# Tyler-Sch/pyruhvro

Measured on AMD Instinct MI355X. Metric: Avro records/sec -> Arrow (direct decode, input and output resident in HBM), higher is better.
Workload: dtype u8

## Files before the change

include/ruhvro_hip.h:

```cpp
#ifndef RUHVRO_HIP_H
#define RUHVRO_HIP_H
#include <stddef.h>
#include <stdint.h>
#include "arrow_c_abi.h"

#ifdef __cplusplus
extern "C" {
#endif

#define RH_ABI_VERSION 7

#define RH_OK 0
#define RH_ERR_SCHEMA 1
#define RH_ERR_DECODE 2
#define RH_ERR_RUNTIME 3
#define RH_ERR_ARGUMENT 4

typedef struct rh_schema rh_schema;

rh_schema* rh_schema_compile(const char* json, size_t len, char** err);
void rh_schema_free(rh_schema* s);

rh_schema* rh_schema_project(const rh_schema* s, const char* const* names, uint32_t n_names, char** err);

// ... 10 lines not shown

typedef struct {
  int32_t device;
  int32_t flags;
  void* stream;
  const int32_t* devices;
  uint32_t n_devices;
  uint32_t struct_size;
  uint64_t chunk_rows;
  rh_stats* device_stats;
  const uint64_t* ready;
  uint64_t* gathered;
} rh_opts;

#define RH_KERNEL_AUTO 0
#define RH_KERNEL_GENERIC 1
#define RH_KERNEL_SPECIALIZED 2
#define RH_ASYNC 8
#define RH_TWO_PASS 16
#define RH_SINGLE_PASS 32

struct rh_stats {
  uint64_t records;
  uint64_t input_bytes;
  uint64_t output_bytes;
  uint32_t chunks;
  uint32_t blocks;
  float pack_ms;
  float h2d_ms;
  float size_kernel_ms;
  float scan_kernel_ms;
  float emit_kernel_ms;
  float d2h_ms;
  float total_ms;
  uint32_t specialized;
  uint32_t lds_bytes;
};

int rh_decode(const rh_schema* s, const uint8_t* const* ptrs, const uint64_t* lens,
              uint64_t n, uint64_t num_chunks, const rh_opts* opts,
              struct ArrowArray* out_chunks, uint32_t* out_k, rh_stats* stats, char** err);

int rh_decode_packed(const rh_schema* s, const uint8_t* data, const uint64_t* offsets,
                     uint64_t n, uint64_t num_chunks, const rh_opts* opts,
                     struct ArrowArray* out_chunks, uint32_t* out_k, rh_stats* stats, char** err);

typedef struct rh_device_result rh_device_result;
int rh_decode_device(const rh_schema* s, const void* d_data, const void* d_offsets,
                     uint64_t data_len, uint64_t n, uint64_t num_chunks, const rh_opts* opts,
                     rh_device_result** out, rh_stats* stats, char** err);
int rh_device_result_wait(rh_device_result* r, rh_stats* stats, char** err);
uint32_t rh_device_result_chunks(const rh_device_result* r);
uint64_t rh_device_result_output_bytes(const rh_device_result* r);
int rh_device_result_export(rh_device_result* r, uint32_t chunk, struct ArrowDeviceArray* out);
uint32_t rh_device_result_buffers(rh_device_result* r, uint32_t chunk, uint64_t* ptrs, uint64_t* sizes, uint32_t cap);
int rh_device_result_to_host(rh_device_result* r, struct ArrowArray* out_chunks, char** err);
void rh_device_result_free(rh_device_result* r);

char* rh_schema_kernel_source(const rh_schema* s);
char* rh_schema_kernel_key(const rh_schema* s, int encode);
char* rh_schema_encode_kernel_source(const rh_schema* s);
int rh_schema_prebuild(const rh_schema* s, int* cached, char** err);
int rh_schema_kernels_ready(const rh_schema* s, int encode, long timeout_ms, char** err);

char* rh_schema_lean_kernel_source(const rh_schema* s);
char* rh_schema_lean_kernel_key(const rh_schema* s);
int rh_schema_lean_ready(const rh_schema* s, long timeout_ms, char** err);
int rh_schema_lean_state(const rh_schema* s, int device);
enum {
  RH_LEAN_CALLS = 0,
  RH_LEAN_PROBES = 1,
  RH_LEAN_PROBES_CLEAN = 2,
  RH_LEAN_PROBES_DIRTY = 3,
  RH_LEAN_FALLBACKS = 4,
  RH_LEAN_RERUNS = 5,
  RH_LEAN_NEED_RANGED = 6,
  RH_LEAN_NEED_WIDE_INDEX = 7,
  RH_LEAN_TWO_PASS_REPEATS = 8,
  RH_LEAN_CAPACITY_TAILS = 9,
  RH_LEAN_ASYNC_SETTLED = 10,
  RH_LEAN_COUNT = 11
};
uint32_t rh_lean_counters(uint64_t* out, uint32_t n);

int rh_encode(const rh_schema* s, const struct ArrowArray* batch, const struct ArrowSchema* batch_schema,
              uint64_t num_chunks, const rh_opts* opts, struct ArrowArray* out_chunks, uint32_t* out_k,
              rh_stats* stats, char** err);

typedef struct rh_device_encoded rh_device_encoded;
int rh_encode_device(const rh_schema* s, const struct ArrowArray* batch, const struct ArrowSchema* batch_schema,
                     uint64_t num_chunks, const rh_opts* opts, rh_device_encoded** out, rh_stats* stats, char** err);
uint32_t rh_device_encoded_chunks(const rh_device_encoded* r);
uint64_t rh_device_encoded_output_bytes(const rh_device_encoded* r);
int rh_device_encoded_export(rh_device_encoded* r, uint32_t chunk, struct ArrowDeviceArray* out);
int rh_device_encoded_to_host(rh_device_encoded* r, struct ArrowArray* out_chunks, char** err);
void rh_device_encoded_free(rh_device_encoded* r);

enum {
  RH_CTR_FUSED_CALLS = 0,
  RH_CTR_TWO_SYNC_CALLS = 1,
  RH_CTR_CAPACITY_RETRIES = 2,
  RH_CTR_WIDE_FALLBACKS = 3,
  RH_CTR_OFFSET32_ERRORS = 4,
  RH_CTR_SPLIT_CALLS = 5,
  RH_CTR_SINGLE_PASS_CALLS = 6,
  RH_CTR_SINGLE_PASS_FAILOVERS = 7,
  RH_CTR_BACKGROUND_COMPILES = 8,
  RH_CTR_TILES = 9,
  RH_CTR_CAREFUL_TILES = 10,
  RH_CTR_OVER_WINDOW_TILES = 11,
  RH_CTR_REWALKED_WAVES = 12,
  RH_CTR_SUBTILED_TILES = 13,
  RH_CTR_RANGED_RETRIES = 14,
  RH_CTR_TOLERANT_CALLS = 15,
  RH_CTR_TOLERANT_REPAIRS = 16,
  RH_CTR_COUNT = 17
};
uint32_t rh_engine_counters(uint64_t* out, uint32_t n);

int rh_schema_placeholder(const rh_schema* s, const uint8_t** bytes, uint64_t* len);
typedef struct rh_record_errors rh_record_errors;
uint64_t rh_record_errors_count(const rh_record_errors* e);
int rh_record_errors_get(const rh_record_errors* e, uint64_t i, uint64_t* index, int* code, const char** message);
void rh_record_errors_free(rh_record_errors* e);
int rh_validate(const rh_schema* s, const uint8_t* const* ptrs, const uint64_t* lens, uint64_t n, const rh_opts* opts,
                uint64_t max_errors, rh_record_errors** out, uint64_t* total_bad, char** err);
int rh_validate_packed(const rh_schema* s, const uint8_t* data, const uint64_t* offsets, uint64_t n, const rh_opts* opts,
                       uint64_t max_errors, rh_record_errors** out, uint64_t* total_bad, char** err);
int rh_validate_device(const rh_schema* s, const void* d_data, const void* d_offsets, uint64_t data_len, uint64_t n,
                       const rh_opts* opts, uint64_t max_errors, rh_record_errors** out, uint64_t* total_bad, char** err);
int rh_decode_tolerant(const rh_schema* s, const uint8_t* const* ptrs, const uint64_t* lens, uint64_t n, uint64_t num_chunks,
                       const rh_opts* opts, struct ArrowArray* out_chunks, uint32_t* out_k, rh_stats* stats, char** err,
                       uint64_t max_errors, rh_record_errors** errors);
int rh_decode_packed_tolerant(const rh_schema* s, const uint8_t* data, const uint64_t* offsets, uint64_t n, uint64_t num_chunks,
                              const rh_opts* opts, struct ArrowArray* out_chunks, uint32_t* out_k, rh_stats* stats, char** err,
                              uint64_t max_errors, rh_record_errors** errors);
int rh_decode_device_tolerant(const rh_schema* s, const void* d_data, const void* d_offsets, uint64_t data_len, uint64_t n,
                              uint64_t num_chunks, const rh_opts* opts, rh_device_result** out, rh_stats* stats, char** err,
                              uint64_t max_errors, rh_record_errors** errors);

typedef struct rh_container_info rh_container_info;
int rh_container_scan(const uint8_t* data, uint64_t len, rh_container_info** info, char** err);
const char* rh_container_info_schema(const rh_container_info* i, uint64_t* len);
const char* rh_container_info_codec(const rh_container_info* i);
const uint8_t* rh_container_info_sync(const rh_container_info* i);
uint64_t rh_container_info_blocks(const rh_container_info* i);
uint64_t rh_container_info_records(const rh_container_info* i);
int rh_container_info_table(const rh_container_info* i, const uint64_t** start, const uint64_t** end, const uint64_t** first);
uint32_t rh_container_info_metadata_count(const rh_container_info* i);
int rh_container_info_metadata_get(const rh_container_info* i, uint32_t k, const char** key, const uint8_t** value, uint64_t* value_len);
void rh_container_info_free(rh_container_info* i);
int rh_decode_blocks(const rh_schema* s, const uint8_t* data, uint64_t len, const uint64_t* start, const uint64_t* end,
                     const uint64_t* first, uint64_t nb, uint64_t num_chunks, const rh_opts* opts, struct ArrowArray* out_chunks,
                     uint32_t* out_k, rh_stats* stats, char** err);
int rh_decode_blocks_device(const rh_schema* s, const uint8_t* data, uint64_t len, const uint64_t* start, const uint64_t* end,
                            const uint64_t* first, uint64_t nb, uint64_t num_chunks, const rh_opts* opts, rh_device_result** out,
                            rh_stats* stats, char** err);
float rh_split_last_ms(void);

uint64_t rh_bench_gather(const uint8_t* const* ptrs, const uint64_t* lens, uint64_t n, uint32_t shards,
                         uint32_t threads_per_shard, int pinned, uint32_t reps, double* best_ms);
uint32_t rh_numa_nodes(void);

uint32_t rh_selftest_pool(uint32_t workers, uint32_t phases, uint32_t max_tasks);

void rh_free_string(char* s);
// ... 10 lines not shown
```

pyruhvro_amd/_build.py:

```python
from __future__ import annotations

import os
import subprocess
import sysconfig

HERE = os.path.dirname(os.path.abspath(__file__))
CSRC = os.path.join(HERE, "csrc")
ROOT = os.path.dirname(HERE)
LIB = os.path.join(HERE, "libruhvro_hip.so")
EXT = os.path.join(HERE, "_pyruhvro.so")

LIB_SOURCES = ["kernels.hip", "encode.hip", "validate.hip", "container.hip", "engine_tolerant.cpp", "engine_container.cpp", "container_scan.cpp", "engine.cpp", "engine_pools.cpp", "engine_kernels.cpp", "engine_device_call.cpp", "engine_host.cpp",
               "engine_export.cpp", "engine_encode.cpp", "schema.cpp", "specialize.cpp", "rtc_compile.cpp", "kernel_jobs.cpp"]
HELPER = os.path.join(HERE, "rh_kcompile")
EMBED = ["program.h", "walk.h", "kernel_common.h", "spec_body.h", "encode.h", "encode_walk.h", "encode_spec.h", "walk_drop.h", "spec_flat.h", "walk_resolve.h"]
LIB_DEPS = LIB_SOURCES + EMBED + ["engine_internal.h", "specialize.h", "rtc_compile.h", "kernel_jobs.h", "kcompile_main.cpp", "schema.h", "validate.h", "container.h", "container_scan.h", "json.hpp", "../../include/ruhvro_hip.h", "../../include/arrow_c_abi.h"]


def _stale(target: str, deps) -> bool:
    if not os.path.exists(target):
        return True
    t = os.path.getmtime(target)
    return any(os.path.getmtime(os.path.join(CSRC, d)) > t for d in deps)


def _embed_headers() -> None:
    out = ["// generated by pyruhvro_amd/_build.py from " + ", ".join(EMBED) + " -- do not edit"]
    for h in EMBED:
        text = open(os.path.join(CSRC, h)).read()
        assert ")RHX\"" not in text
        out.append("static const char kHdr_%s[] = R\"RHX(%s)RHX\";" % (h.replace(".", "_"), text))
    path = os.path.join(CSRC, "embedded_headers.inc")
    new = "\n".join(out) + "\n"
    if not os.path.exists(path) or open(path).read() != new:
        open(path, "w").write(new)


def _prune_kernel_cache() -> None:
    d = os.path.join(HERE, "_kcache")
    if os.path.isdir(d):
        for f in os.listdir(d):
            if f.endswith((".hsaco", ".tmp", ".ok", ".lock", ".src", ".err")):
                try:
                    os.remove(os.path.join(d, f))
                except OSError:
                    pass


def _compile_objects(verbose: bool = False):
    from concurrent.futures import ThreadPoolExecutor
    objdir = os.path.join(HERE, "build")
    os.makedirs(objdir, exist_ok=True)
    inc = ["-I", os.path.join(ROOT, "include")]
    clang = "/opt/rocm/lib/llvm/bin/clang++"
    jobs = []
    for src in LIB_SOURCES:
        obj = os.path.join(objdir, os.path.splitext(src)[0] + ".o")
        if src.endswith(".hip") or not os.path.exists(clang):
            cmd = ["hipcc", "--offload-arch=gfx950", "-O3", "-std=c++17", "-fPIC", "-w"] + inc + ["-c", os.path.join(CSRC, src), "-o", obj]
        else:
            cmd = [clang, "-O3", "-std=c++17", "-fPIC", "-w", "-D__HIP_PLATFORM_AMD__", "-I", "/opt/rocm/include"] + inc + \
                  ["-c", os.path.join(CSRC, src), "-o", obj]
        jobs.append((cmd, obj))

    def run(job):
        if verbose:
            print(" ".join(job[0]))
        subprocess.check_call(job[0])
        return job[1]

    with ThreadPoolExecutor(max_workers=min(len(jobs), os.cpu_count() or 2)) as ex:
        return list(ex.map(run, jobs))


def build_lib(force: bool = False, verbose: bool = False) -> str:
    if force or _stale(LIB, LIB_DEPS):
        _embed_headers()
        objs = _compile_objects(verbose)
        cmd = ["hipcc", "--offload-arch=gfx950", "-fPIC", "-shared"] + objs + ["-o", LIB + ".tmp", "-lpthread", "-ldl"]
        if verbose:
            print(" ".join(cmd))
        subprocess.check_call(cmd)
        os.replace(LIB + ".tmp", LIB)
        for o in objs:
            os.remove(o)
        build_helper(verbose)
        _prune_kernel_cache()
    elif not os.path.exists(HELPER):
        build_helper(verbose)
    return LIB


def build_helper(verbose: bool = False) -> str:
    _embed_headers()
    cmd = ["g++", "-O2", "-std=c++17", "-w", os.path.join(CSRC, "kcompile_main.cpp"), os.path.join(CSRC, "rtc_compile.cpp"),
           "-o", HELPER + ".tmp", "-ldl", "-lpthread"]
    if verbose:
        print(" ".join(cmd))
# ... 68 lines not shown
```

pyruhvro_amd/cabi.py:

```python
from __future__ import annotations

import ctypes as C
import os
from collections import namedtuple
from typing import List, Optional

import numpy as np
import pyarrow as pa

_HERE = os.path.dirname(os.path.abspath(__file__))
LIB_PATH = os.environ.get("RUHVRO_HIP_LIB") or os.path.join(_HERE, "libruhvro_hip.so")

RH_OK, RH_ERR_SCHEMA, RH_ERR_DECODE, RH_ERR_RUNTIME, RH_ERR_ARGUMENT = range(5)


class RhStats(C.Structure):
    _fields_ = [("records", C.c_uint64), ("input_bytes", C.c_uint64), ("output_bytes", C.c_uint64),
                ("chunks", C.c_uint32), ("blocks", C.c_uint32), ("pack_ms", C.c_float), ("h2d_ms", C.c_float),
                ("size_kernel_ms", C.c_float), ("scan_kernel_ms", C.c_float), ("emit_kernel_ms", C.c_float),
                ("d2h_ms", C.c_float), ("total_ms", C.c_float), ("specialized", C.c_uint32), ("lds_bytes", C.c_uint32)]

    def as_dict(self):
        return {n: getattr(self, n) for n, _ in self._fields_}

# ... 239 lines not shown
KERNEL_AUTO, KERNEL_GENERIC, KERNEL_SPECIALIZED = 0, 1, 2
RH_TWO_PASS = 16
RH_SINGLE_PASS = 32
RH_ASYNC = 8


def kernel_source(schema_json: str, columns=None, reader_schema=None) -> str:
    L = lib()
    p = L.rh_schema_kernel_source(Schema.get(schema_json, columns, reader_schema).handle)
    if not p:
        raise RuntimeError("rh_schema_kernel_source failed")
    try:
        return C.string_at(p).decode()
    finally:
        L.rh_free_string(p)


def kernel_key(schema_json: str, encode: bool = False, columns=None, reader_schema=None) -> str:
    L = lib()
    p = L.rh_schema_kernel_key(Schema.get(schema_json, columns, reader_schema).handle, 1 if encode else 0)
    if not p:
        raise RuntimeError("rh_schema_kernel_key failed")
    try:
        return C.string_at(p).decode()
    finally:
        L.rh_free_string(p)


LEAN_COUNTERS = ("lean_calls", "probes", "probes_clean", "probes_dirty", "fallbacks", "reruns", "need_ranged", "need_wide_index",
                 "two_pass_repeats", "capacity_tails", "async_settled")
LEAN_NONE, LEAN_UNDECIDED, LEAN_LEAN, LEAN_WIDE = -1, 0, 1, 2


def _lean_sym(name: str, restype, argtypes):
    f = getattr(lib(), name, None)
    if f is not None:
        f.restype, f.argtypes = restype, argtypes
    return f


def _lean_string(name: str, schema_json: str, columns=None, reader_schema=None):
    f = _lean_sym(name, C.c_void_p, [C.c_void_p])
    p = f(Schema.get(schema_json, columns, reader_schema).handle) if f else None
    if not p:
        return None
    try:
        return C.string_at(p).decode()
    finally:
        lib().rh_free_string(p)


def lean_kernel_source(schema_json: str, columns=None, reader_schema=None):
    return _lean_string("rh_schema_lean_kernel_source", schema_json, columns, reader_schema)


def lean_kernel_key(schema_json: str, columns=None, reader_schema=None):
    return _lean_string("rh_schema_lean_kernel_key", schema_json, columns, reader_schema)


def lean_state(schema_json: str, device: int = 0, columns=None, reader_schema=None) -> int:
    f = _lean_sym("rh_schema_lean_state", C.c_int, [C.c_void_p, C.c_int])
    return int(f(Schema.get(schema_json, columns, reader_schema).handle, device)) if f else LEAN_NONE


def lean_ready(schema_json: str, timeout_ms: int = 0) -> bool:
    f = _lean_sym("rh_schema_lean_ready", C.c_int, [C.c_void_p, C.c_long, C.POINTER(C.c_char_p)])
    if f is None:
        return False
    err = C.c_char_p()
    rc = f(Schema.get(schema_json).handle, int(timeout_ms), C.byref(err))
    if rc == -1:
        _raise(RH_ERR_RUNTIME, err)
    return rc == 1


def lean_counters() -> dict:
    f = _lean_sym("rh_lean_counters", C.c_uint32, [C.POINTER(C.c_uint64), C.c_uint32])
    buf = (C.c_uint64 * len(LEAN_COUNTERS))()
    if f is not None:
        assert f(buf, len(LEAN_COUNTERS)) == len(LEAN_COUNTERS)
    return {name: int(buf[i]) for i, name in enumerate(LEAN_COUNTERS)}


def encode_kernel_source(schema_json: str) -> str:
    L = lib()
    p = L.rh_schema_encode_kernel_source(Schema.get(schema_json).handle)
    if not p:
        raise RuntimeError("rh_schema_encode_kernel_source failed")
    try:
        return C.string_at(p).decode()
    finally:
        L.rh_free_string(p)


def prebuild(schema_json: str, columns=None, reader_schema=None) -> bool:
    L = lib()
    cached = C.c_int()
    err = C.c_char_p()
    rc = L.rh_schema_prebuild(Schema.get(schema_json, columns, reader_schema).handle, C.byref(cached), C.byref(err))
    if rc != RH_OK:
        _raise(rc, err)
    return bool(cached.value)


def kernels_ready(schema_json: str, encode: bool = False, timeout_ms: int = 0, columns=None, reader_schema=None) -> bool:
    err = C.c_char_p()
    rc = lib().rh_schema_kernels_ready(Schema.get(schema_json, columns, reader_schema).handle, 1 if encode else 0, int(timeout_ms), C.byref(err))
    if rc < 0:
        _raise(RH_ERR_RUNTIME, err)
    return rc == 1


def shard_chunks(n: int, num_chunks: int, n_shards: int, shard: int):
    c0, c1, r0, r1 = C.c_uint32(), C.c_uint32(), C.c_uint64(), C.c_uint64()
    lib().rh_shard_chunks(n, num_chunks, n_shards, shard, C.byref(c0), C.byref(c1), C.byref(r0), C.byref(r1))
    return c0.value, c1.value, r0.value, r1.value


def decode_packed(data: np.ndarray, offsets: np.ndarray, schema_json: str, num_chunks: int,
                  device: int = -1, want_stats: bool = False, kernel: int = KERNEL_AUTO, devices=None, *, columns=None, reader_schema=None):
    L = lib()
    s = Schema.get(schema_json, columns, reader_schema)
    data = np.ascontiguousarray(data, dtype=np.uint8)
    offsets = np.ascontiguousarray(offsets, dtype=np.uint64)
    n = len(offsets) - 1
    k = L.rh_clamp_chunks(n, num_chunks)
    arr = (ArrowArray * k)()
    out_k = C.c_uint32()
    st = RhStats()
    err = C.c_char_p()
    opts, keep = make_opts(device, kernel, None, devices)
    rc = L.rh_decode_packed(s.handle, data.ctypes.data, offsets.ctypes.data, n, num_chunks, C.byref(opts), arr,
                            C.byref(out_k), C.byref(st), C.byref(err))
    if rc != RH_OK:
        _raise(rc, err)
    out = _import_chunks(arr, out_k.value, s.arrow_schema)
    if not want_stats:
        return out
    d = st.as_dict()
    if devices:
        d["device_stats"] = [x.as_dict() for x in keep["device_stats"]]
    return out, d


def decode_slices(ptrs: np.ndarray, lens: np.ndarray, schema_json: str, num_chunks: int,
                  device: int = -1, want_stats: bool = False, kernel: int = KERNEL_AUTO, devices=None, *, columns=None, reader_schema=None):
    L = lib()
    s = Schema.get(schema_json, columns, reader_schema)
    ptrs = np.ascontiguousarray(ptrs, dtype=np.uint64)
    lens = np.ascontiguousarray(lens, dtype=np.uint64)
    n = len(ptrs)
    k = L.rh_clamp_chunks(n, num_chunks)
    arr = (ArrowArray * k)()
    out_k = C.c_uint32()
    st = RhStats()
    err = C.c_char_p()
    opts, keep = make_opts(device, kernel, None, devices)
    rc = L.rh_decode(s.handle, ptrs.ctypes.data, lens.ctypes.data, n, num_chunks, C.byref(opts), arr,
                     C.byref(out_k), C.byref(st), C.byref(err))
    if rc != RH_OK:
        _raise(rc, err)
    out = _import_chunks(arr, out_k.value, s.arrow_schema)
    return (out, st.as_dict()) if want_stats else out


RecordError = namedtuple("RecordError", ["index", "message"])
# ... 391 lines not shown
```

pyruhvro_amd/csrc/engine.cpp:

```cpp
#include "engine_internal.h"

#include <sched.h>

using namespace rhe;

bool stats_line_on() {
  static const bool on = [] { const char* e = std::getenv("RUHVRO_HIP_STATS"); return e && *e && *e != '0'; }();
  return on;
}
void stats_json(std::string& o, const rh_stats& st) {
  char buf[512];
  std::snprintf(buf, sizeof buf,
                "{\"records\": %llu, \"input_bytes\": %llu, \"output_bytes\": %llu, \"chunks\": %u, \"blocks\": %u, \"pack_ms\": %.4f, "
                "\"h2d_ms\": %.4f, \"size_kernel_ms\": %.4f, \"scan_kernel_ms\": %.4f, \"emit_kernel_ms\": %.4f, \"d2h_ms\": %.4f, "
                "\"total_ms\": %.4f, \"specialized\": %u, \"lds_bytes\": %u}",
                (unsigned long long)st.records, (unsigned long long)st.input_bytes, (unsigned long long)st.output_bytes, st.chunks,
                st.blocks, st.pack_ms, st.h2d_ms, st.size_kernel_ms, st.scan_kernel_ms, st.emit_kernel_ms, st.d2h_ms, st.total_ms,
                st.specialized, st.lds_bytes);
  o += buf;
}
void stats_line(const char* entry, int rc, const rh_stats& st, const rh_opts* opts, const rh_stats* shards) {
  std::string o = "{\"ruhvro_hip\": \"";
  o += entry;
  o += "\", \"rc\": " + std::to_string(rc) + ", \"stats\": ";
// ... 198 lines not shown
  return RH_OK;
}

int rh_decode_device(const rh_schema* s, const void* d_data, const void* d_offsets, uint64_t data_len, uint64_t n,
                     uint64_t num_chunks, const rh_opts* opts, rh_device_result** out, rh_stats* stats, char** err) {
  if (!s || !out) return RH_ERR_ARGUMENT;
  return guarded(err, [&] {
    require_device();
    Timer t;
    rh_opts pub;
    if (opts) { pub = *opts; pub.flags &= kPublicFlags; }
    *out = decode_device_impl(const_cast<rh_schema*>(s), (const uint8_t*)d_data, (const uint64_t*)d_offsets, data_len,
                              n, num_chunks, opts ? &pub : nullptr, stats);
    if (stats) stats->total_ms = t.ms();
    return RH_OK;
  });
}

char* rh_schema_kernel_source(const rh_schema* s) {
  if (!s) return nullptr;
  try {
    return dup_msg(rh::generate_kernel_source(*s->cs));
  } catch (...) {
    return nullptr;
  }
}

char* rh_schema_kernel_key(const rh_schema* s, int encode) {
  if (!s) return nullptr;
  try {
    if (encode && (!s->cs->encode_unsupported.empty() || s->cs->projected)) return nullptr;
    const std::string src = encode ? rh::generate_encode_source(*s->cs) : rh::generate_kernel_source(*s->cs);
    return dup_msg(rh::kernel_cache_key(src, encode != 0));
  } catch (...) {
    return nullptr;
  }
}

char* rh_schema_lean_kernel_source(const rh_schema* s) {
  if (!s) return nullptr;
  try {
    const std::string src = rh::generate_lean_source(*s->cs);
    return src.empty() ? nullptr : dup_msg(src);
  } catch (...) {
    return nullptr;
  }
}

char* rh_schema_lean_kernel_key(const rh_schema* s) {
  if (!s) return nullptr;
  try {
    const std::string src = rh::generate_lean_source(*s->cs);
    return src.empty() ? nullptr : dup_msg(rh::kernel_cache_key(src, false));
  } catch (...) {
    return nullptr;
  }
}

int rh_schema_lean_ready(const rh_schema* s, long timeout_ms, char** err) {
  if (!s) return -1;
  try {
    if (!rh::schema_has_lean(*s->cs)) return -2;
    rh::KernelImage im[rh::KP_COUNT];
    rh::kernel_images(s->images, *s->cs, rh::kLeanParts, rh::CP_CACHED_ONLY, im);
    std::string why;
    const int rc = rh::kernel_images_wait(s->images, rh::kLeanParts, timeout_ms, &why);
    if (rc < 0 && err) *err = dup_msg(why);
    return rc;
  } catch (const std::exception& e) {
    if (err) *err = dup_msg(e.what());
    return -1;
  }
}

int rh_schema_lean_state(const rh_schema* cs_, int device) {
  rh_schema* s = const_cast<rh_schema*>(cs_);
  if (!s) return -1;
  if (!rh::schema_has_lean(*s->cs)) return -1;
  std::lock_guard<std::mutex> g(s->mu);
  auto it = s->spec.find(device);
  return (it == s->spec.end() || !it->second) ? 0 : it->second->lean_state;
}

char* rh_schema_encode_kernel_source(const rh_schema* s) {
  if (!s || !s->cs->encode_unsupported.empty() || s->cs->projected) return nullptr;
  try {
    return dup_msg(rh::generate_encode_source(*s->cs));
  } catch (...) {
    return nullptr;
  }
}

int rh_schema_prebuild(const rh_schema* s, int* cached, char** err) {
  if (!s) return RH_ERR_ARGUMENT;
  return guarded(err, [&] {
    const bool fused = env_long("RUHVRO_HIP_PREBUILD_FUSED", 1, 0, 1) != 0;
    const bool ranged = env_long("RUHVRO_HIP_PREBUILD_RANGED", 1, 0, 1) != 0;
    const bool lean = env_long("RUHVRO_HIP_PREBUILD_LEAN", 0, 0, 1) != 0;
    const unsigned parts = (rh::kDecodeParts & ~(fused ? 0u : (1u << rh::KP_FUSED)) & ~(ranged ? 0u : ((1u << rh::KP_SIZE_R) | (1u << rh::KP_EMIT_R)))) |
                           ((s->cs->encode_unsupported.empty() && !s->cs->wide && !s->cs->projected) ? rh::kEncodeParts : 0u) |
                           (lean ? rh::kLeanParts : 0u);
    rh::KernelImage im[rh::KP_COUNT];
    const unsigned started = rh::kernel_images(s->images, *s->cs, parts, rh::CP_BLOCKING, im);
    for (int p = 0; p < rh::KP_COUNT; p++) {
      if (!(parts & (1u << p)) || im[p].state == rh::IMG_NONE) continue;
      if (im[p].state != rh::IMG_READY) throw std::runtime_error(std::string(rh::kernel_part_entry(p)) + ": " + (im[p].why.empty() ? "kernel image missing" : im[p].why));
    }
    if (cached) *cached = started == 0 ? 1 : 0;
    return RH_OK;
  });
}

int rh_schema_kernels_ready(const rh_schema* s, int encode, long timeout_ms, char** err) {
  if (!s) return -1;
  try {
    if (encode && s->cs->projected) {
      if (err) *err = dup_msg(s->cs->resolved ? "a resolved schema is decode only" : "a projected schema is decode only");
      return -1;
    }
    const unsigned parts = encode ? rh::kEncodeParts : ((1u << rh::KP_SIZE) | (1u << rh::KP_EMIT));
    rh::KernelImage im[rh::KP_COUNT];
    rh::kernel_images(s->images, *s->cs, parts, rh::CP_CACHED_ONLY, im);
    std::string why;
    const int rc = rh::kernel_images_wait(s->images, parts, timeout_ms, &why);
    if (rc < 0 && err) *err = dup_msg(why);
    return rc;
  } catch (const std::exception& e) {
    if (err) *err = dup_msg(e.what());
    return -1;
  }
}

uint32_t rh_device_result_chunks(const rh_device_result* r) { return r ? r->k : 0; }

uint64_t rh_device_result_output_bytes(const rh_device_result* r) {
  if (!r) return 0;
  try {
    settle(const_cast<rh_device_result*>(r));
    if (!r->parts.empty()) {
      uint64_t sum = 0;
      for (auto& p : r->parts) { p->tables(); sum += p->output_bytes; }
      return sum;
    }
    const_cast<rh_device_result*>(r)->tables();
  } catch (...) {
    return 0;
  }
  return r->output_bytes;
}

int rh_device_result_wait(rh_device_result* r, rh_stats* stats, char** err) {
  if (!r) return RH_ERR_ARGUMENT;
  return guarded(err, [&] {
    settle(r);
    if (stats && r->has_stats) *stats = r->st;
    return RH_OK;
  });
}

int rh_device_result_export(rh_device_result* r, uint32_t chunk, struct ArrowDeviceArray* out) {
  if (!r || !out || chunk >= r->k) return RH_ERR_ARGUMENT;
  std::memset(out, 0, sizeof *out);
  try {
    settle(r);
    rh_device_result* owner = r;
    for (size_t g = 0; g < r->parts.size(); g++)
      if (chunk >= r->part_chunk0[g] && chunk < r->part_chunk0[g] + r->parts[g]->k) { owner = r->parts[g].get(); chunk -= r->part_chunk0[g]; break; }
    owner->tables();
    export_chunk(*owner, chunk, owner->arena.ptr(), nullptr, &out->array);
  } catch (const DecodeError&) {
    return RH_ERR_DECODE;
  } catch (...) {
    return RH_ERR_RUNTIME;
  }
  out->device_id = r->device;
  out->device_type = ARROW_DEVICE_ROCM;
  out->sync_event = nullptr;
  return RH_OK;
}

uint32_t rh_device_result_buffers(rh_device_result* r, uint32_t chunk, uint64_t* ptrs, uint64_t* sizes, uint32_t cap) {
  if (!r || chunk >= r->k) return 0;
  try {
    settle(r);
// ... 51 lines not shown
```

pyruhvro_amd/csrc/engine_device_call.cpp:

```cpp
#include "engine_internal.h"

using namespace rhe;

struct rh_decode_call {
  rh_schema* s;
  const CompiledSchema& cs;
  const uint8_t* d_data;
  const uint64_t* d_offsets;
  uint64_t data_len, n, num_chunks;
  rh_opts opts;
  bool want_stats;
  rh_stats st;
  rh_device_result& r;
  HostProf hp;
  int device = 0;
  hipStream_t stream = nullptr;
  ChunkGeo geo_v;
  const ChunkGeo* geo = nullptr;
  uint32_t k = 1;
  int K = 0, nnodes = 0, nbuf = 0;
  const DeviceProgram* dp = nullptr;
  const SpecKernel* sk = nullptr;
  hipFunction_t size_r = nullptr, emit_r = nullptr;
  hipFunction_t size_f = nullptr, emit_f = nullptr;
  hipFunction_t lean_size = nullptr, lean_emit = nullptr;
  bool lean = false;
  bool probing = false;
  uint32_t probe_token = 0;
  Lease probe_ws, probe_host;
  std::unique_ptr<CtrlLease> probe_ctrl;
  uint64_t narrow_rows = 0, tile = 0, bpc64 = 0, payload = 0;
  uint32_t nblocks = 0;
  uint64_t o_null = 0, o_tot = 48, ctrl_bytes = 0;
  uint32_t null_slots = rh::kNullSlots;
  Lease ws, hctrl, dtab, prof_buf;
  std::unique_ptr<CtrlLease> ctrl;
  rh::KParams P;
  uint32_t lds_bytes = 0, emit_lds = 0;
  bool profile = false;
  Events ev;
  std::vector<uint64_t> totals;
  uint64_t n_entries = 0, tab_bytes = 0;
  uint64_t* d_sizes = nullptr;
  uint64_t exact = 0;
  bool child_bitmaps = false, fused = false, timed_size = false;
  bool range_of_host_call = false;
  bool single = false;
  std::vector<uint64_t> caps;
  uint64_t arena_cap = 0, o_tick = 0;
  Lease lookback, hcaps;
  double basis = 0;
  bool settled = false;
  bool async = false;
  DoneEvent done;
  hipEvent_t start_after = nullptr, sized = nullptr;
  bool published = false;
  uint32_t token = 0;
  uint64_t o_flag_h = 0;

  rh_decode_call(rh_schema* s_, const uint8_t* data, const uint64_t* offs, uint64_t dl, uint64_t n_, uint64_t nc, const rh_opts* o,
               bool stats, const ChunkGeo* g, rh_device_result& res)
      : s(s_), cs(*s_->cs), d_data(data), d_offsets(offs), data_len(dl), n(n_), num_chunks(nc), opts(o ? *o : default_opts()),
        want_stats(stats), r(res) {
    std::memset(&st, 0, sizeof st);
    if (g) { geo_v = *g; geo = &geo_v; range_of_host_call = true; }
    opts.devices = nullptr; opts.n_devices = 0; opts.device_stats = nullptr; opts.ready = nullptr; opts.gathered = nullptr;
  }

  Lease arena_lease(uint64_t bytes) {
    r.arena_host = false;
    if ((opts.flags & RH_INTERNAL_HOST_ARENA) && !child_bitmaps && env_long("RUHVRO_HIP_HOST_ARENA", 1, 0, 1) != 0) {
      Block b = pin_pool().try_get(bytes, device);
      if (b.p) {
        r.arena_host = true;
        return Lease(pin_pool(), b);
      }
      pin_pool().prefetch(bytes + bytes / 16, device, pinned_budget_left());
    }
    return Lease(dev_pool(), bytes, device);
  }

  void check_bad(const uint8_t* h) {
    unsigned long long fb = *(const unsigned long long*)h;
    if (!fb) return;
    const uint64_t rec = ~fb;
    uint64_t c = r.sz ? std::min<uint64_t>(rec / r.sz, k - 1) : 0;
    uint64_t b = c * bpc64 + (rec - c * r.sz) / tile;
    rh::ErrInfo ei;
    HIPCHK(hipMemcpy(&ei, P.errinfo + b, sizeof ei, hipMemcpyDeviceToHost));
    throw RecordDecodeError(format_error(ei));
  }

  void learn_unsized_tiles() {
    if (timed_size || single || n == 0) return;
    const uint32_t* stw = (const uint32_t*)(hctrl.ptr() + 32);
    count(RH_CTR_OVER_WINDOW_TILES, stw[1]); count(RH_CTR_SUBTILED_TILES, stw[3]);
    if (stw[1]) s->ranged_calls.store(kRangedKeep, std::memory_order_relaxed);
    else { uint32_t v = s->ranged_calls.load(std::memory_order_relaxed); if (v) s->ranged_calls.compare_exchange_weak(v, v - 1, std::memory_order_relaxed); }
  }

  void layout_host() {
    r.data_bytes = totals;
    for (auto t : totals)
      if (t > 0x7FFFFFFFull) {
        count(RH_CTR_OFFSET32_ERRORS);
        throw DecodeError("offset overflow: a chunk's column exceeds the 2^31-1 limit of 32-bit Arrow offsets");
      }
    if (sk)
      for (int d = 1; d < cs.ndom; d++)
        for (uint32_t c = 0; c < k; c++)
          if (totals[(size_t)(d - 1) * k + c] >= narrow_rows) {
            if (lean) lean_count(LC_NEED_WIDE_INDEX);
            throw NeedWideIndex();
          }
    r.fill_tables();
    exact = r.output_bytes;
  }

  void launch_tail(bool offsets_done) {
    if (nbuf > 0 && (child_bitmaps || !offsets_done) &&
        rh_launch_init(P.bufptr, d_sizes, dp->desc, (uint32_t)nbuf, k, P.first_bad, stream)) throw HipError("k_init launch failed");
    if (n > 0) {
      emit_lds = lds_bytes;
      if (sk ? launch_module(emit_f, P, nblocks, (uint32_t)tile, emit_lds, stream, ev.at(3), P.ranged ? nullptr : ev.at(4))
             : (cs.projected ? rh_launch_emit_drop : rh_launch_emit)(&P, emit_lds, stream, ev.at(3), ev.at(4)))
        throw HipError("k_emit launch failed");
      if (P.ranged && launch_module(emit_r, P, nblocks + (P.worklist ? rh::kBigFront : 0u), (uint32_t)tile, emit_lds, stream, nullptr, ev.at(4))) throw HipError("k_emit (ranged) launch failed");
    } else {
      ev.rec(3, stream);
      ev.rec(4, stream);
// ... 52 lines not shown
    const uint64_t rows_lastp = kp == k ? r.rows_last : r.sz;
    const uint32_t tiles_last = (uint32_t)std::min<uint64_t>(per, (rows_lastp + tile - 1) / tile);
    if (per == 0 || tiles_last == 0) return;
    const uint32_t pn = (kp - 1) * per + tiles_last;
    {
      std::lock_guard<std::mutex> g(s->mu);
      SpecKernel& sl = sel();
      if (sl.lean_state == SpecKernel::LS_LEAN || sl.lean_probing) return;
      if (sl.lean_state == SpecKernel::LS_WIDE && sl.lean_wait > 0) { sl.lean_wait--; return; }
      sl.lean_probing = true;
    }
    probing = true;
    const uint64_t q_bsum = align_up(sizeof(rh::ErrInfo) * (uint64_t)pn, kAlign);
    const uint64_t q_flag = align_up(q_bsum + 4ull * std::max(K, 1) * pn, kAlign);
    const uint64_t q_lcnt = align_up(q_flag + 4ull * pn, kAlign);
    const uint64_t q_end = align_up(q_lcnt + 4ull * (uint64_t)((cs.KL + 1) / 2) * pn * tile, kAlign) + kAlign;
    probe_ws = Lease(dev_pool(), q_end, device);
    probe_host = Lease(pin_pool(), 256, device);
    probe_ctrl.reset(new CtrlLease(ctrl_bytes, device, stream));
    void* hdev = nullptr;
    if (hipHostGetDevicePointer(&hdev, probe_host.ptr(), 0) != hipSuccess || !hdev) {
      (void)hipGetLastError();
      probe_abandon();
      return;
    }
    rh::KParams Q = P;
    Q.k = kp; Q.rows_last = rows_lastp; Q.bpc = per; Q.nblocks = pn;
    Q.ranged = 0; Q.worklist = nullptr; Q.bigmark = nullptr; Q.all_careful = 0; Q.lookback = nullptr; Q.caps = nullptr;
    Q.first_bad = (unsigned long long*)probe_ctrl->ptr();
    Q.nullcount = (uint32_t*)(probe_ctrl->ptr() + o_null);
    Q.totals = (uint64_t*)(probe_ctrl->ptr() + o_tot);
    Q.tickets = (uint32_t*)(probe_ctrl->ptr() + o_tick);
    Q.errinfo = (rh::ErrInfo*)probe_ws.ptr();
    Q.blocksum = (uint32_t*)(probe_ws.ptr() + q_bsum);
    Q.blockbase = Q.blocksum;
    Q.tileflag = (uint32_t*)(probe_ws.ptr() + q_flag);
    Q.lanecnt = (uint32_t*)(probe_ws.ptr() + q_lcnt);
    Q.lanecnt32 = nullptr;
    static std::atomic<uint32_t> next_token{0x20000001u};
    probe_token = next_token.fetch_add(1);
    if (probe_token == 0) probe_token = next_token.fetch_add(1);
    *(volatile uint32_t*)(probe_host.ptr() + 48) = 0;
    if (launch_module(lean_size, Q, pn, (uint32_t)tile, lds_bytes, stream) ||
        rh_launch_tile_stats(probe_ctrl->ptr(), Q.tileflag, pn, stream) ||
        rh_launch_publish(probe_ctrl->ptr(), hdev, 12, 0, 12, probe_token, null_slots, stream))
      throw HipError("lean probe launch failed");
  }

  void probe_abandon() noexcept {
    if (!probing) return;
    probing = false;
    std::lock_guard<std::mutex> g(s->mu);
    sel().lean_probing = false;
  }

  void probe_settle() {
    if (!probing) return;
    volatile uint32_t* flag = (volatile uint32_t*)(probe_host.ptr() + 48);
    bool got = true;
    for (uint32_t spins = 0; __atomic_load_n(flag, __ATOMIC_ACQUIRE) != probe_token;) {
      if ((++spins & 0xFFFFu) == 0) {
        const hipError_t q = hipStreamQuery(stream);
        if (q == hipErrorNotReady) continue;
        got = __atomic_load_n(flag, __ATOMIC_ACQUIRE) == probe_token;
        break;
      }
    }
    const uint32_t* h = (const uint32_t*)probe_host.ptr();
    const bool clean = got && h[0] == 0 && h[1] == 0 && h[2] == 0 && h[8] == 0 && h[9] == 0 && h[10] == 0;
    lean_count(LC_PROBES);
    lean_count(clean ? LC_PROBES_CLEAN : LC_PROBES_DIRTY);
    {
      std::lock_guard<std::mutex> g(s->mu);
      SpecKernel& sl = sel();
      sl.lean_probing = false;
      if (clean) sl.lean_state = SpecKernel::LS_LEAN;
      else { sl.lean_state = SpecKernel::LS_WIDE; sl.lean_wait = 64; }
    }
    probing = false;
    if (got) { probe_ws.release(); probe_host.release(); probe_ctrl.reset(); }
  }

  void lean_learn(bool dirty) {
    if (!lean) return;
    std::lock_guard<std::mutex> g(s->mu);
    SpecKernel& sl = sel();
    if (dirty) {
      if (sl.lean_state != SpecKernel::LS_WIDE) {
        sl.lean_backoff = std::min<uint32_t>(1024, std::max<uint32_t>(8, sl.lean_backoff * 2));
        sl.lean_wait = sl.lean_backoff;
        sl.lean_state = SpecKernel::LS_WIDE;
        lean_count(LC_FALLBACKS);
      }
    } else if (sl.lean_state == SpecKernel::LS_LEAN) {
      sl.lean_backoff = 0;
    }
  }

  bool try_single(bool two_sync, long ratio_hook) {
    const bool on = (opts.flags & RH_SINGLE_PASS) != 0 || env_long("RUHVRO_HIP_SINGLE_PASS", kSinglePassDefault, 0, 1) != 0;
    if (!on || range_of_host_call || (opts.flags & (RH_INTERNAL_TWO_PASS | RH_TWO_PASS)) || !sk || K <= 0 || K > 64 || n == 0 || two_sync ||
        ratio_hook >= 0)
      return false;
    if (n_entries > (1u << 16)) return false;
    if (8ull * K * k > 4ull * K * nblocks) return false;
    hipFunction_t fused_fn = sk->fused_fn.load(std::memory_order_acquire);
    if (!fused_fn) {
      if (sk->fused_dead) return false;
      fused_fn = spec_kernel(s, device, compile_policy(opts.flags & 3, n), false, true).fused_fn.load(std::memory_order_acquire);
      if (!fused_fn) return false;
    }
    std::vector<double> per_row;
    {
      std::lock_guard<std::mutex> g(s->mu);
      if ((int)s->per_row.size() != K) return false;
      if (s->single_cooldown > 0) { s->single_cooldown--; return false; }
      per_row = s->per_row;
    }
    const double slack = (double)env_long("RUHVRO_HIP_SINGLE_SLACK_PERMILLE", 1040, 1, 4000) / 1000.0;
    caps.assign((size_t)K * k, 0);
    for (int kk = 0; kk < K; kk++)
      for (uint32_t c = 0; c < k; c++) {
        const uint64_t rows_c = c == k - 1 ? r.rows_last : r.sz;
        uint64_t cap = (uint64_t)(per_row[(size_t)kk] * (double)rows_c * slack) + (slack >= 1.0 ? 4096 : 0);
        uint64_t lim = 0x7FFFFFFFull;
        if (kk < cs.ndom - 1) lim = std::min<uint64_t>(lim, narrow_rows - 1);
        caps[(size_t)kk * k + c] = std::min(cap, lim);
      }
    {
      uint64_t off = 0;
      for (uint32_t c = 0; c < k; c++)
        for (int b = 0; b < nbuf; b++) {
          const rh::BufDesc& d = cs.bufs[b];
          const uint64_t rows0 = c == k - 1 ? r.rows_last : r.sz;
          const uint64_t rows = d.dom == 0 ? rows0 : caps[(size_t)(d.dom - 1) * k + c];
          off += rh::buf_slot_bytes(rh::buf_bytes(d.kind, rows, d.kind == rh::BK_DATA ? caps[(size_t)d.counter * k + c] : 0, nullptr, (uint32_t)d.counter));
        }
      arena_cap = std::max<uint64_t>(off, kAlign);
    }
    count(RH_CTR_SINGLE_PASS_CALLS);
    count(RH_CTR_FUSED_CALLS);
    single = true; fused = true;
    r.arena = Lease(dev_pool(), arena_cap, device);
    lookback = Lease(dev_pool(), std::max<uint64_t>(8ull * K * nblocks, kAlign), device);
    HIPCHK(hipMemsetAsync(lookback.ptr(), 0, 8ull * K * nblocks, stream));
    hcaps = Lease(pin_pool(), 8ull * K * k, device);
    std::memcpy(hcaps.ptr(), caps.data(), 8ull * K * k);
    uint64_t* d_caps = (uint64_t*)P.blocksum;
    HIPCHK(hipMemcpyAsync(d_caps, hcaps.ptr(), 8ull * K * k, hipMemcpyHostToDevice, stream));
    P.lookback = (unsigned long long*)lookback.ptr();
    P.caps = d_caps;
    rh::LParams LP;
    std::memset(&LP, 0, sizeof LP);
    LP.totals = d_caps; LP.desc = dp->desc; LP.sz = r.sz; LP.rows_last = r.rows_last; LP.n = n; LP.k = k;
    LP.nbuf = nbuf; LP.K = K; LP.ndom = cs.ndom; LP.arena = r.arena.ptr(); LP.capacity = r.arena.b.size;
    LP.bufptr = (void**)dtab.ptr(); LP.bufsize = d_sizes; LP.ctrl = P.first_bad; LP.narrow = 0;
    LP.narrow_rows = narrow_rows;
    if (rh_launch_layout(&LP, stream)) throw HipError("k_layout launch failed");
    if (nbuf > 0 && child_bitmaps && rh_launch_init(P.bufptr, d_sizes, dp->desc, (uint32_t)nbuf, k, P.first_bad, stream))
      throw HipError("k_init launch failed");
    const uint64_t tiles_max = std::max<uint64_t>((r.sz + tile - 1) / tile, (r.rows_last + tile - 1) / tile);
    emit_lds = lds_bytes;
    if (launch_module(fused_fn, P, (uint32_t)(tiles_max * k), (uint32_t)tile, emit_lds, stream, ev.at(3), ev.at(4)))
      throw HipError("k_fused launch failed");
    basis = (double)payload + 64.0 * (double)n;
    void* hdev = nullptr;
    if (hipHostGetDevicePointer(&hdev, hctrl.ptr(), 0) == hipSuccess && hdev) {
      static std::atomic<uint32_t> next_token{0x40000001u};
      token = next_token.fetch_add(1);
      if (token == 0) token = next_token.fetch_add(1);
      o_flag_h = align_up(o_null + 4ull * nnodes * k, 8);
      *(volatile uint32_t*)(hctrl.ptr() + o_flag_h) = 0;
      if (rh_launch_publish(ctrl->ptr(), hdev, (uint32_t)(o_null / 4), (uint32_t)(nnodes * (int)k), (uint32_t)(o_flag_h / 4), token, null_slots, stream))
        throw HipError("k_publish launch failed");
      ctrl->b.clean = true;
      published = true;
    } else {
      (void)hipGetLastError();
      HIPCHK(hipMemcpyAsync(hctrl.ptr(), ctrl->ptr(), ctrl_bytes, hipMemcpyDeviceToHost, stream));
      if (async) done.record(device, stream);
    }
    return true;
  }

  void enqueue() {
    Range rk("ruhvro_hip:decode_device (k_size, k_scan, k_layout, k_init, k_emit)");
    if (opts.device >= 0) { HIPCHK(hipSetDevice(opts.device)); device = opts.device; }
    else HIPCHK(hipGetDevice(&device));
    stream = (hipStream_t)opts.stream;
    if ((uintptr_t)d_data & 15) throw std::invalid_argument("device payload pointer must be 16-byte aligned");

    {
      static std::mutex lds_mu;
      static std::vector<int> lds_done;
      std::lock_guard<std::mutex> g(lds_mu);
      if (std::find(lds_done.begin(), lds_done.end(), device) == lds_done.end()) {
        if (rh_set_max_lds(160 * 1024) != 0) throw HipError("cannot raise the dynamic LDS limit of the decode kernels");
        lds_done.push_back(device);
      }
    }

    r.cs = &cs;
    r.device = device;
    r.n = n;
    if (!geo && opts.chunk_rows) {
      if (num_chunks < 1 || num_chunks > 0xFFFFFFFFull || (num_chunks - 1) > n / opts.chunk_rows ||
          (n > 0 && n == (num_chunks - 1) * opts.chunk_rows && num_chunks > 1))
        throw std::invalid_argument("chunk_rows: the n records do not make num_chunks chunks of chunk_rows rows (the last one takes the rest)");
      geo_v.k = (uint32_t)num_chunks;
      geo_v.sz = opts.chunk_rows;
      geo_v.rows_last = n - (num_chunks - 1) * opts.chunk_rows;
      geo_v.payload_bytes = data_len;
      geo = &geo_v;
    }
    k = geo ? geo->k : rh_clamp_chunks(n, num_chunks);
    r.k = k;
    r.sz = geo ? geo->sz : n / k;
    r.rows_last = geo ? geo->rows_last : n - (uint64_t)(k - 1) * r.sz;
    K = cs.K; nnodes = (int)cs.nodes.size(); nbuf = (int)cs.bufs.size();
    dp = &device_program(s, device);

    const int mode = opts.flags & 3;
// ... 152 lines not shown
      const uint64_t capacity = align_up((uint64_t)(ratio * basis * 1.125) + n_entries * kAlign + (1u << 20), kAlign);
      r.arena = arena_lease(capacity);
      rh::LParams LP;
      std::memset(&LP, 0, sizeof LP);
      LP.totals = P.totals; LP.desc = dp->desc; LP.sz = r.sz; LP.rows_last = r.rows_last; LP.n = n; LP.k = k;
      LP.nbuf = nbuf; LP.K = K; LP.ndom = cs.ndom; LP.arena = r.arena.ptr(); LP.capacity = r.arena.b.size;
      LP.bufptr = (void**)dtab.ptr(); LP.bufsize = d_sizes; LP.ctrl = P.first_bad; LP.narrow = sk ? 1u : 0u;
      LP.narrow_rows = narrow_rows;
      if (timed_size && K == 0 && rh_launch_tile_stats(ctrl->ptr(), P.tileflag, nblocks, stream)) throw HipError("k_tile_stats launch failed");
      if ((timed_size && K > 0) ? rh_launch_scan_layout(&P, &LP, stream, ev.at(5), ev.at(2)) : rh_launch_layout(&LP, stream))
        throw HipError("k_scan / k_layout launch failed");
      launch_tail(true);
      hp.mark("layout+emit_launch");
      void* hdev = nullptr;
      static const bool no_publish = env_long("RUHVRO_HIP_NO_PUBLISH", 0, 0, 1) != 0;
      if (!no_publish && hipHostGetDevicePointer(&hdev, hctrl.ptr(), 0) == hipSuccess && hdev) {
        static std::atomic<uint32_t> next_token{1};
        token = next_token.fetch_add(1);
        if (token == 0) token = next_token.fetch_add(1);
        o_flag_h = align_up(o_null + 4ull * nnodes * k, 8);
        *(volatile uint32_t*)(hctrl.ptr() + o_flag_h) = 0;
        if (rh_launch_publish(ctrl->ptr(), hdev, (uint32_t)(o_null / 4), (uint32_t)(nnodes * (int)k), (uint32_t)(o_flag_h / 4), token, null_slots, stream))
          throw HipError("k_publish launch failed");
        ctrl->b.clean = true;
        published = true;
      } else {
        (void)hipGetLastError();
        HIPCHK(hipMemcpyAsync(hctrl.ptr(), ctrl->ptr(), ctrl_bytes, hipMemcpyDeviceToHost, stream));
        if (async) done.record(device, stream);
      }
      hp.mark("d2h_enqueue");
    }
    launch_probe();
  }

  void finish() {
    if (settled) return;
    settled = true;
    HIPCHK(hipSetDevice(device));
    if (fused) {
      if (published) {
        volatile uint32_t* flag = (volatile uint32_t*)(hctrl.ptr() + o_flag_h);
        for (uint32_t spins = 0; __atomic_load_n(flag, __ATOMIC_ACQUIRE) != token;) {
          if ((++spins & 0xFFFFu) == 0) {
            const hipError_t q = hipStreamQuery(stream);
            if (q == hipSuccess) {
              if (__atomic_load_n(flag, __ATOMIC_ACQUIRE) != token) throw HipError("rh_k_publish finished without publishing its token");
              break;
            }
            if (q != hipErrorNotReady) throw HipError(std::string("stream failed while waiting for a decode call: ") + hipGetErrorString(q));
          }
#if defined(__x86_64__)
          __builtin_ia32_pause();
#endif
        }
      } else if (done.e) {
        done.wait();
      } else {
        HIPCHK(hipStreamSynchronize(stream));
      }
      hp.mark("sync");
      probe_settle();
      const uint32_t lflag = *(const uint32_t*)(hctrl.ptr() + 8);
      if (lflag & rh::LF_NEED_RANGED) {
        ctrl->b.clean = published;
        s->ranged_calls.store(kRangedKeep, std::memory_order_relaxed);
        r.arena.release();
        if (lean) { lean_count(LC_NEED_RANGED); lean_learn(true); }
        throw NeedRanged();
      }
      check_bad(hctrl.ptr());
      if (lean && !single) { const uint32_t* stw = (const uint32_t*)(hctrl.ptr() + 32); lean_learn(stw[0] != 0 || stw[2] != 0); }
      if (published && timed_size && !single) {
        const uint32_t* stw = (const uint32_t*)(hctrl.ptr() + 32);
        count(RH_CTR_TILES, nblocks);
        count(RH_CTR_CAREFUL_TILES, stw[0]); count(RH_CTR_OVER_WINDOW_TILES, stw[1]);
        count(RH_CTR_REWALKED_WAVES, stw[2]); count(RH_CTR_SUBTILED_TILES, stw[3]);
        if (stw[1]) s->ranged_calls.store(kRangedKeep, std::memory_order_relaxed);
        else { uint32_t v = s->ranged_calls.load(std::memory_order_relaxed); if (v) s->ranged_calls.compare_exchange_weak(v, v - 1, std::memory_order_relaxed); }
      }
      if (K > 0) std::memcpy(totals.data(), hctrl.ptr() + o_tot, 8ull * K * k);
      if (single) {
        ctrl->b.clean = published;
        if (lflag) {
          if ((lflag & rh::LF_CAPACITY) && env_long("RUHVRO_HIP_SINGLE_SLACK_PERMILLE", 1040, 1, 4000) >= 1000) {
            std::lock_guard<std::mutex> g(s->mu);
            s->single_backoff = std::min<uint32_t>(1024, std::max<uint32_t>(8, s->single_backoff * 2));
            s->single_cooldown = s->single_backoff;
          }
          count(RH_CTR_SINGLE_PASS_FAILOVERS);
          r.arena.release();
          throw NeedTwoPass();
        }
        r.data_bytes = totals;
        r.layout_bytes = caps;
        r.arena_bytes = arena_cap;
        { std::lock_guard<std::mutex> g(s->mu); s->single_backoff = 0; }
      } else if (lflag & rh::LF_CAPACITY) {
        count(RH_CTR_CAPACITY_RETRIES);
        if (lean) lean_count(LC_CAPACITY_TAILS);
        r.arena.release();
        exact_tail();
      } else if (lflag || want_stats) {
        layout_host();
        if (lflag) throw HipError("internal error: layout kernel and host disagree");
        if (r.arena_bytes != std::max<uint64_t>(*(const uint64_t*)(hctrl.ptr() + 16), kAlign)) throw HipError("internal error: device and host arena layouts differ");
      } else {
        r.data_bytes = totals;
        r.arena_bytes = std::max<uint64_t>(*(const uint64_t*)(hctrl.ptr() + 16), kAlign);
      }
    } else {
      count(RH_CTR_TWO_SYNC_CALLS);
      if (timed_size) {
        HIPCHK(hipMemcpyAsync(hctrl.ptr(), ctrl->ptr(), ctrl_bytes, hipMemcpyDeviceToHost, stream));
        HIPCHK(hipStreamSynchronize(stream));
        probe_settle();
        if (*(const uint32_t*)(hctrl.ptr() + 8) & rh::LF_NEED_RANGED) {
          ctrl->b.clean = false;
          s->ranged_calls.store(kRangedKeep, std::memory_order_relaxed);
          throw NeedRanged();
        }
        check_bad(hctrl.ptr());
        std::memcpy(totals.data(), hctrl.ptr() + o_tot, 8ull * K * k);
      }
      exact_tail();
    }
    learn_unsized_tiles();
    if (n > 0 && basis > 0 && !single) {
      const double slots = (double)n_entries * (double)kAlign;
      s->arena_ratio.store(std::max(0.0, (double)r.arena_bytes - slots) / basis + 1e-9);
    }
    if (n > 0 && K > 0 && (int)totals.size() == K * (int)k) {
      std::vector<double> pr((size_t)K, 0.0);
      for (int kk = 0; kk < K; kk++)
        for (uint32_t c = 0; c < k; c++) {
          const uint64_t rows_c = c == k - 1 ? r.rows_last : r.sz;
          if (rows_c) pr[(size_t)kk] = std::max(pr[(size_t)kk], (double)totals[(size_t)kk * k + c] / (double)rows_c);
        }
      std::lock_guard<std::mutex> g(s->mu);
      s->per_row = std::move(pr);
    }
    r.nullcount.assign((size_t)nnodes * k, 0);
    if (published) {
      std::memcpy(r.nullcount.data(), hctrl.ptr() + o_null, 4ull * nnodes * k);
    } else {
      const uint32_t* slots = (const uint32_t*)(hctrl.ptr() + o_null);
      for (size_t e = 0; e < (size_t)nnodes * k; e++) {
        uint32_t sum = 0;
        for (uint32_t sl = 0; sl < null_slots; sl++) sum += slots[e * null_slots + sl];
        r.nullcount[e] = sum;
      }
    }
    hp.mark("host_layout");

    if (profile && sk) {
      unsigned long long hr[64 * 32], h[32] = {0};
      HIPCHK(hipMemcpy(hr, prof_buf.ptr(), sizeof hr, hipMemcpyDeviceToHost));
      for (int r0 = 0; r0 < 64; r0++)
        for (int i = 0; i < 32; i++) h[i] += hr[r0 * 32 + i];
      const double waves = (double)nblocks * 4;
      static const char* names2[] = {"offsets", "stage+barrier", "lane_init", "walk1", "scan", "barrier", "layout", "walk2",
                                     "errors+barrier", "flush"};
      static const char* names1[] = {"ticket+zero+barrier", "offsets+stage+barrier", "size_walk", "wave_scan", "barrier", "lookback(wave0)",
                                     "barrier", "prefix", "emit_walk", "errors+flush"};
      const char* const* names = single ? names1 : names2;
      std::fprintf(stderr, "[ruhvro_hip profile] %s cycles/wave:", single ? "single-pass" : "emit");
// ... 288 lines not shown
```

pyruhvro_amd/csrc/engine_internal.h:

```cpp
#pragma once
#include <hip/hip_runtime_api.h>
#include <dlfcn.h>
#include <pthread.h>

extern "C" hipError_t hipExtModuleLaunchKernel(hipFunction_t f, uint32_t globalWorkSizeX, uint32_t globalWorkSizeY,
                                               uint32_t globalWorkSizeZ, uint32_t localWorkSizeX, uint32_t localWorkSizeY,
                                               uint32_t localWorkSizeZ, size_t sharedMemBytes, hipStream_t hStream,
                                               void** kernelParams, void** extra, hipEvent_t startEvent,
                                               hipEvent_t stopEvent, uint32_t flags);

#include <algorithm>
#include <atomic>
#include <chrono>
#include <cstdio>
#include <cstdlib>
#include <cstring>
#include <functional>
#include <map>
#include <condition_variable>
#include <mutex>
#include <string>
#include <thread>
#include <vector>

// ... 192 lines not shown
  uint64_t cached_ = 0;
};

Pool& dev_pool();
Pool& pin_pool();

struct Lease {
  Pool* pool = nullptr;
  Block b;
  Lease() = default;
  Lease(Pool& p, uint64_t size, int device) : pool(&p), b(p.get(size, device)) {}
  Lease(Pool& p, Block taken) : pool(&p), b(taken) {}
  Lease(const Lease&) = delete;
  Lease& operator=(const Lease&) = delete;
  Lease(Lease&& o) noexcept : pool(o.pool), b(o.b) { o.pool = nullptr; o.b = Block(); }
  Lease& operator=(Lease&& o) noexcept {
    if (this != &o) { release(); pool = o.pool; b = o.b; o.pool = nullptr; o.b = Block(); }
    return *this;
  }
  ~Lease() { release(); }
  void release() { if (pool && b.p) pool->put(b); pool = nullptr; b = Block(); }
  uint8_t* ptr() const { return (uint8_t*)b.p; }
};

class CtrlPool {
 public:
  struct Blk { void* p = nullptr; uint64_t size = 0; int device = 0; hipStream_t stream = nullptr; bool clean = false; };
  Blk get(uint64_t size, int device, hipStream_t stream) {
    size = align_up(std::max<uint64_t>(size, 1), 4096);
    {
      std::lock_guard<std::mutex> g(mu_);
      for (size_t i = 0; i < free_.size(); i++)
        if (free_[i].device == device && free_[i].stream == stream && free_[i].size == size) {
          Blk b = free_[i];
          free_.erase(free_.begin() + (long)i);
          return b;
        }
    }
    Blk b;
    b.size = size; b.device = device; b.stream = stream;
    hipError_t e = hipMalloc(&b.p, size);
    if (e != hipSuccess) throw HipError(std::string("HIP allocation of a control block failed: ") + hipGetErrorString(e));
    e = hipMemsetAsync(b.p, 0, size, stream);
    if (e != hipSuccess) { (void)hipFree(b.p); throw HipError(std::string("hipMemsetAsync failed: ") + hipGetErrorString(e)); }
    return b;
  }
  void put(Blk b) {
    if (!b.p) return;
    if (!b.clean && hipMemsetAsync(b.p, 0, b.size, b.stream) != hipSuccess) { (void)hipFree(b.p); return; }
    b.clean = false;
    Blk drop;
    {
      std::lock_guard<std::mutex> g(mu_);
      free_.push_back(b);
      if (free_.size() > 64) { drop = free_.front(); free_.erase(free_.begin()); }
    }
    if (drop.p) (void)hipFree(drop.p);
  }

 private:
  std::mutex mu_;
  std::vector<Blk> free_;
};
CtrlPool& ctrl_pool();

struct CtrlLease {
  CtrlPool::Blk b;
  CtrlLease(uint64_t size, int device, hipStream_t stream) : b(ctrl_pool().get(size, device, stream)) {}
  CtrlLease(const CtrlLease&) = delete;
  CtrlLease& operator=(const CtrlLease&) = delete;
  ~CtrlLease() { ctrl_pool().put(b); }
  uint8_t* ptr() const { return (uint8_t*)b.p; }
};

struct DeviceProgram {
  rh::Op* prog = nullptr;
  uint32_t* sym_off = nullptr;
  uint8_t* sym_data = nullptr;
  rh::BufDesc* desc = nullptr;
  int32_t* cnt_databuf = nullptr;
};

struct SpecKernel {
  hipModule_t mod[7] = {nullptr, nullptr, nullptr, nullptr, nullptr, nullptr, nullptr};
  hipFunction_t size_fn = nullptr, emit_fn = nullptr;
  std::atomic<hipFunction_t> size_r_fn{nullptr}, emit_r_fn{nullptr};
  std::atomic<bool> ranged_dead{false};
  std::atomic<hipFunction_t> size_l_fn{nullptr}, emit_l_fn{nullptr};
  std::atomic<bool> lean_dead{false};
  enum : int { LS_UNDECIDED = 0, LS_LEAN = 1, LS_WIDE = 2 };
  int lean_state = LS_UNDECIDED;
  uint32_t lean_wait = 0;
  uint32_t lean_backoff = 0;
  bool lean_probing = false;
  std::atomic<hipFunction_t> fused_fn{nullptr};
  std::atomic<bool> fused_dead{false};
  std::atomic<bool> ok{false};
  std::atomic<bool> dead{false};
  std::string why;
};

}

struct rh_schema {
  std::unique_ptr<rh::CompiledSchema> cs;
  std::mutex mu;
  std::map<int, rhe::DeviceProgram> dev;
  std::map<int, std::unique_ptr<rhe::SpecKernel>> spec;
  std::map<int, std::unique_ptr<rhe::SpecKernel>> espec;
  std::shared_ptr<rh::KernelImages> images = rh::new_kernel_images();
  std::atomic<double> arena_ratio{0.0};
  std::vector<double> per_row;
  std::atomic<uint32_t> ranged_calls{0};
  std::vector<uint8_t> placeholder;
  bool placeholder_done = false;
  rh_schema* plain_parent = nullptr;
  uint32_t single_cooldown = 0, single_backoff = 0;
};

namespace rhe {

const DeviceProgram& device_program(rh_schema* s, int device);
uint64_t spec_min_records();
const SpecKernel& spec_kernel(rh_schema* s, int device, rh::CompilePolicy policy, bool encode = false, bool want_fused = false, bool want_ranged = false,
                              bool want_lean = false);
enum LeanCounter { LC_LEAN_CALLS = 0, LC_PROBES, LC_PROBES_CLEAN, LC_PROBES_DIRTY, LC_FALLBACKS, LC_RERUNS, LC_NEED_RANGED, LC_NEED_WIDE_INDEX,
                   LC_TWO_PASS_REPEATS, LC_CAPACITY_TAILS, LC_ASYNC_SETTLED, LC_COUNT };
extern std::atomic<uint64_t> g_lean_counters[LC_COUNT];
inline void lean_count(int which, uint64_t by = 1) { g_lean_counters[which].fetch_add(by, std::memory_order_relaxed); }
rh::CompilePolicy compile_policy(int mode, uint64_t n);
int launch_module(hipFunction_t f, const rh::KParams& P, uint32_t grid, uint32_t block, uint32_t lds, hipStream_t stream,
                  hipEvent_t start = nullptr, hipEvent_t stop = nullptr);
std::string format_error(const rh::ErrInfo& e);

struct Roctx {
  int (*push)(const char*) = nullptr;
  int (*pop)() = nullptr;
  Roctx() {
    const char* e = std::getenv("RUHVRO_HIP_ROCTX");
    const bool want = e && *e && *e != '0';
    for (const char* name : {"librocprofiler-sdk-roctx.so.1", "libroctx64.so.4", "librocprofiler-sdk-roctx.so", "libroctx64.so"}) {
      void* h = dlopen(name, RTLD_LAZY | RTLD_NOLOAD);
      if (!h && want) h = dlopen(name, RTLD_LAZY);
      if (!h) continue;
      push = (int (*)(const char*))dlsym(h, "roctxRangePushA");
      pop = (int (*)())dlsym(h, "roctxRangePop");
      if (push && pop) return;
      push = nullptr; pop = nullptr;
    }
  }
  static const Roctx& get() { static const Roctx r; return r; }
};
struct Range {
  bool on;
  explicit Range(const char* name) : on(Roctx::get().push != nullptr) { if (on) Roctx::get().push(name); }
  ~Range() { if (on) Roctx::get().pop(); }
  Range(const Range&) = delete;
  Range& operator=(const Range&) = delete;
};

struct HostProf {
  bool on;
  std::chrono::steady_clock::time_point t0;
  std::string line;
  HostProf() {
    static const bool e = [] { const char* v = std::getenv("RUHVRO_HIP_HOSTPROF"); return v && *v && *v != '0'; }();
    on = e;
    if (on) t0 = std::chrono::steady_clock::now();
  }
  void mark(const char* what) {
    if (!on) return;
    const auto t = std::chrono::steady_clock::now();
    char buf[64];
    std::snprintf(buf, sizeof buf, " %s=%.1f", what, std::chrono::duration<double, std::micro>(t - t0).count());
    line += buf;
    t0 = t;
  }
  ~HostProf() { if (on) std::fprintf(stderr, "[ruhvro_hip hostprof us]%s\n", line.c_str()); }
};

struct Timeline {
  static bool on() {
    static const bool e = [] { const char* v = std::getenv("RUHVRO_HIP_TIMELINE"); return v && *v && *v != '0'; }();
    return e;
  }
  static std::chrono::steady_clock::time_point& t0() {
    static std::chrono::steady_clock::time_point t = std::chrono::steady_clock::now();
    return t;
  }
  static void start() { if (on()) t0() = std::chrono::steady_clock::now(); }
  static void mark(uint32_t shard, const char* what) {
    if (!on()) return;
    std::fprintf(stderr, "[ruhvro_hip timeline] %8.3f ms  shard %u  %s\n",
                 std::chrono::duration<double, std::milli>(std::chrono::steady_clock::now() - t0()).count(), shard, what);
  }
};

inline rh_opts default_opts() {
  rh_opts o;
  std::memset(&o, 0, sizeof o);
  o.device = -1;
  return o;
}

struct Timer {
  std::chrono::steady_clock::time_point t0 = std::chrono::steady_clock::now();
  float ms() const { return std::chrono::duration<float, std::milli>(std::chrono::steady_clock::now() - t0).count(); }
};
// ... 2 lines not shown

struct rh_decode_call;
struct rh_device_result {
  const rh::CompiledSchema* cs = nullptr;
  int device = 0;
  uint64_t n = 0, sz = 0, rows_last = 0;
  uint32_t k = 1;
  rhe::Lease arena;
  bool arena_host = false;
  uint64_t arena_bytes = 0;
  std::vector<uint64_t> buf_off;
  std::vector<uint64_t> buf_size;
  std::vector<uint64_t> dom_rows;
  std::vector<uint64_t> data_bytes;
  std::vector<uint64_t> layout_bytes;
  std::vector<uint32_t> nullcount;
  uint64_t output_bytes = 0;
  std::mutex tables_mu;
  bool tables_done = false;
  std::unique_ptr<rh_decode_call> pending;
  std::exception_ptr fail;
  rh_stats st;
  bool has_stats = false;
  std::vector<std::unique_ptr<rh_device_result>> parts;
  std::vector<uint32_t> part_chunk0;
  rhe::Lease patched_data, patched_offsets;
  rhe::Lease container_data, container_offsets;
  std::vector<hipEvent_t> join_events;

  rh_device_result();
  ~rh_device_result();
  uint64_t rows(int dom, uint32_t c) const { return dom_rows[(size_t)dom * k + c]; }
  void fill_tables();
  void tables() { std::lock_guard<std::mutex> g(tables_mu); if (!tables_done) fill_tables(); }
};

struct rh_device_encoded {
  int device = 0;
  uint64_t n = 0, sz = 0, rows_last = 0;
  uint32_t k = 1;
  rhe::Lease out;
  uint64_t out_bytes = 0;
  std::vector<uint64_t> ooff;
  std::vector<uint64_t> data_bytes;
  uint64_t exact = 0;
  uint64_t rows(uint32_t c) const { return n == 0 ? 0 : (c == k - 1 ? rows_last : sz); }
};

namespace rhe {

struct Slab {
  std::atomic<int> refs{0};
  void* base = nullptr;
  Block pinned;
  void free_mem() {
    if (pinned.p) {
      pinned_result_bytes().fetch_sub(pinned.size);
      pin_pool().put(pinned);
    } else {
      std::free(base);
    }
    pinned = Block();
    base = nullptr;
  }
  static std::atomic<uint64_t>& pinned_result_bytes() {
    static std::atomic<uint64_t> v{0};
    return v;
  }
};

inline uint64_t pinned_budget_left() {
  static const uint64_t bound = (uint64_t)env_long_early("RUHVRO_HIP_PINNED_RESULT_MB", 4096, 0, 1 << 20) << 20;
  const uint64_t used = Slab::pinned_result_bytes().load();
  return used >= bound ? 0 : bound - used;
}

void export_chunk(const rh_device_result& r, uint32_t c, const uint8_t* base, Slab* slab, ArrowArray* out);
void export_field(const rh::ArrowField& f, ArrowSchema* out);
Slab* slab_from_device(const uint8_t* dptr, uint64_t bytes, int device, hipStream_t stream = nullptr);
int to_host_impl(rh_device_result* r, ArrowArray* out_chunks, hipStream_t stream = nullptr);
void settle(rh_device_result* r);

constexpr long kSinglePassDefault = 0;
constexpr int kPublicFlags = 3 | RH_ASYNC | RH_TWO_PASS | RH_SINGLE_PASS;
constexpr int RH_INTERNAL_HOST_ARENA = 0x200;
constexpr int RH_INTERNAL_TWO_PASS = 0x100;
constexpr long kInternalStreamsDefault = 1;
constexpr long kSplitMinDefault = 1000000;

inline long env_long(const char* name, long dflt, long lo, long hi) {
  const char* e = std::getenv(name);
  if (!e || !*e) return dflt;
  char* end = nullptr;
  const long v = std::strtol(e, &end, 10);
  return (end && *end == 0 && v >= lo && v <= hi) ? v : dflt;
}

struct Events {
  hipEvent_t e[6] = {nullptr, nullptr, nullptr, nullptr, nullptr, nullptr};
  bool on = false;
  int device = 0;
  static std::mutex& mu() { static std::mutex m; return m; }
  static std::map<int, std::vector<hipEvent_t>>& idle() { static auto* v = new std::map<int, std::vector<hipEvent_t>>(); return *v; }
  void init() {
    HIPCHK(hipGetDevice(&device));
    {
      std::lock_guard<std::mutex> g(mu());
      auto& v = idle()[device];
      for (auto& x : e)
        if (!v.empty()) { x = v.back(); v.pop_back(); }
    }
    for (auto& x : e)
      if (!x) HIPCHK(hipEventCreate(&x));
    on = true;
  }
  ~Events() {
    if (!on) return;
    std::lock_guard<std::mutex> g(mu());
    auto& v = idle()[device];
    for (auto& x : e) {
      if (!x) continue;
      if (v.size() < 64) v.push_back(x);
      else (void)hipEventDestroy(x);
    }
  }
  void rec(int i, hipStream_t s) { if (on) HIPCHK(hipEventRecord(e[i], s)); }
  hipEvent_t at(int i) const { return on ? e[i] : nullptr; }
  float ms(int a, int b) {
    float t = 0;
    if (on && hipEventElapsedTime(&t, e[a], e[b]) != hipSuccess) { t = 0; (void)hipGetLastError(); }
    return t;
  }
};

struct DoneEvent {
  hipEvent_t e = nullptr;
  int device = 0;
  static std::mutex& mu() { static std::mutex m; return m; }
  static std::map<int, std::vector<hipEvent_t>>& idle() { static auto* v = new std::map<int, std::vector<hipEvent_t>>(); return *v; }
  void record(int dev, hipStream_t s) {
    device = dev;
    {
      std::lock_guard<std::mutex> g(mu());
      auto& v = idle()[device];
      if (!v.empty()) { e = v.back(); v.pop_back(); }
    }
    if (!e) HIPCHK(hipEventCreateWithFlags(&e, hipEventDisableTiming));
    HIPCHK(hipEventRecord(e, s));
  }
  void wait() { if (e) HIPCHK(hipEventSynchronize(e)); }
  ~DoneEvent() {
    if (!e) return;
    std::lock_guard<std::mutex> g(mu());
    auto& v = idle()[device];
    if (v.size() < 64) v.push_back(e);
    else (void)hipEventDestroy(e);
  }
};

struct ChunkGeo {
  uint64_t sz, rows_last;
  uint32_t k;
  uint64_t payload_bytes;
};

rh_device_result* decode_device_impl1(rh_schema* s, const uint8_t* d_data, const uint64_t* d_offsets, uint64_t data_len,
// ... 49 lines not shown
```

pyruhvro_amd/csrc/engine_kernels.cpp:

```cpp
#include "engine_internal.h"

namespace rhe {

const DeviceProgram& device_program(rh_schema* s, int device) {
  std::lock_guard<std::mutex> g(s->mu);
  auto it = s->dev.find(device);
  if (it != s->dev.end()) return it->second;
  const CompiledSchema& cs = *s->cs;
  DeviceProgram d;
  const size_t pb = cs.prog.size() * sizeof(rh::Op), so = cs.sym_off.size() * 4, sd = cs.sym_data.size(),
               bd = std::max<size_t>(cs.bufs.size(), 1) * sizeof(rh::BufDesc);
  HIPCHK(hipMalloc((void**)&d.prog, pb));
  HIPCHK(hipMalloc((void**)&d.sym_off, so));
  HIPCHK(hipMalloc((void**)&d.sym_data, sd));
  HIPCHK(hipMalloc((void**)&d.desc, bd));
  HIPCHK(hipMemcpy(d.prog, cs.prog.data(), pb, hipMemcpyHostToDevice));
  HIPCHK(hipMemcpy(d.sym_off, cs.sym_off.data(), so, hipMemcpyHostToDevice));
  HIPCHK(hipMemcpy(d.sym_data, cs.sym_data.data(), sd, hipMemcpyHostToDevice));
  if (!cs.bufs.empty()) HIPCHK(hipMemcpy(d.desc, cs.bufs.data(), cs.bufs.size() * sizeof(rh::BufDesc), hipMemcpyHostToDevice));
  std::vector<int32_t> cdb((size_t)std::max(cs.K, 1), -1);
  for (size_t b = 0; b < cs.bufs.size(); b++)
    if (cs.bufs[b].kind == rh::BK_DATA) cdb[cs.bufs[b].counter] = (int32_t)b;
  HIPCHK(hipMalloc((void**)&d.cnt_databuf, cdb.size() * 4));
  HIPCHK(hipMemcpy(d.cnt_databuf, cdb.data(), cdb.size() * 4, hipMemcpyHostToDevice));
  return s->dev.emplace(device, d).first->second;
}

uint64_t spec_min_records() {
  static const uint64_t v = [] {
    const char* e = std::getenv("RUHVRO_HIP_SPECIALIZE_MIN");
    return e ? (uint64_t)std::strtoull(e, nullptr, 10) : (uint64_t)32768;
  }();
  return v;
}

hipFunction_t load_part(SpecKernel& k, int slot, const rh::KernelImage& im, int part) {
  hipError_t e = hipModuleLoadData(&k.mod[slot], im.code->data());
  if (e != hipSuccess) throw std::runtime_error(std::string("hipModuleLoadData: ") + hipGetErrorString(e));
  hipFunction_t fn = nullptr;
  e = hipModuleGetFunction(&fn, k.mod[slot], rh::kernel_part_entry(part));
  if (e != hipSuccess) throw std::runtime_error(std::string("hipModuleGetFunction: ") + hipGetErrorString(e));
  (void)hipFuncSetAttribute(reinterpret_cast<const void*>(fn), hipFuncAttributeMaxDynamicSharedMemorySize, 160 * 1024);
  (void)hipGetLastError();
  return fn;
}

const SpecKernel& spec_kernel(rh_schema* s, int device, rh::CompilePolicy policy, bool encode, bool want_fused, bool want_ranged, bool want_lean) {
  std::map<int, std::unique_ptr<SpecKernel>>& table = encode ? s->espec : s->spec;
  SpecKernel* k = nullptr;
  {
    std::lock_guard<std::mutex> g(s->mu);
    std::unique_ptr<SpecKernel>& slot = table[device];
    if (!slot) slot.reset(new SpecKernel);
    k = slot.get();
    if (k->dead) return *k;
    if (k->ok && (!want_fused || k->fused_dead || k->fused_fn.load(std::memory_order_acquire)) &&
        (!want_ranged || k->ranged_dead || k->emit_r_fn.load(std::memory_order_acquire)) &&
        (!want_lean || k->lean_dead || k->emit_l_fn.load(std::memory_order_acquire))) return *k;
  }
  const int p_size = encode ? rh::KP_ESIZE : rh::KP_SIZE, p_emit = encode ? rh::KP_EEMIT : rh::KP_EMIT;
  const unsigned parts = (1u << p_size) | (1u << p_emit) | ((want_fused && !encode) ? (1u << rh::KP_FUSED) : 0u) |
                         ((want_ranged && !encode) ? ((1u << rh::KP_SIZE_R) | (1u << rh::KP_EMIT_R)) : 0u) |
                         ((want_lean && !encode) ? rh::kLeanParts : 0u);
  rh::KernelImage im[rh::KP_COUNT];
  const unsigned started = rh::kernel_images(s->images, *s->cs, parts, policy, im);
  if (started && policy == rh::CP_BACKGROUND) g_counters[RH_CTR_BACKGROUND_COMPILES].fetch_add(started, std::memory_order_relaxed);
  std::lock_guard<std::mutex> g(s->mu);
  if (k->dead) return *k;
  try {
    if (!k->ok) {
      for (int p : {p_size, p_emit})
        if (im[p].state == rh::IMG_FAILED || im[p].state == rh::IMG_NONE) {
          k->dead = true;
          k->why = im[p].state == rh::IMG_NONE ? std::string("the schema has no such kernel") : im[p].why;
          return *k;
        }
      if (im[p_size].state == rh::IMG_READY && im[p_emit].state == rh::IMG_READY) {
        k->size_fn = load_part(*k, 0, im[p_size], p_size);
        k->emit_fn = load_part(*k, 1, im[p_emit], p_emit);
        k->ok = true;
        k->why.clear();
      } else {
        k->why = (im[p_size].state == rh::IMG_COMPILING || im[p_emit].state == rh::IMG_COMPILING) ? "compiling" : "not cached";
      }
    }
    if (k->ok && want_fused && !encode && !k->fused_dead && !k->fused_fn.load(std::memory_order_relaxed)) {
      const rh::KernelImage& f = im[rh::KP_FUSED];
      if (f.state == rh::IMG_FAILED || f.state == rh::IMG_NONE) k->fused_dead = true;
      else if (f.state == rh::IMG_READY) k->fused_fn.store(load_part(*k, 2, f, rh::KP_FUSED), std::memory_order_release);
    }
    if (k->ok && want_ranged && !encode && !k->ranged_dead && !k->emit_r_fn.load(std::memory_order_relaxed)) {
      const rh::KernelImage& a = im[rh::KP_SIZE_R], & b = im[rh::KP_EMIT_R];
      if (a.state == rh::IMG_FAILED || a.state == rh::IMG_NONE || b.state == rh::IMG_FAILED || b.state == rh::IMG_NONE) k->ranged_dead = true;
      else if (a.state == rh::IMG_READY && b.state == rh::IMG_READY) {
        k->size_r_fn.store(load_part(*k, 3, a, rh::KP_SIZE_R), std::memory_order_release);
        k->emit_r_fn.store(load_part(*k, 4, b, rh::KP_EMIT_R), std::memory_order_release);
      }
    }
    if (k->ok && want_lean && !encode && !k->lean_dead && !k->emit_l_fn.load(std::memory_order_relaxed)) {
      const rh::KernelImage& a = im[rh::KP_SIZE_L], & b = im[rh::KP_EMIT_L];
      if (a.state == rh::IMG_FAILED || a.state == rh::IMG_NONE || b.state == rh::IMG_FAILED || b.state == rh::IMG_NONE) k->lean_dead = true;
      else if (a.state == rh::IMG_READY && b.state == rh::IMG_READY) {
        k->size_l_fn.store(load_part(*k, 5, a, rh::KP_SIZE_L), std::memory_order_release);
        k->emit_l_fn.store(load_part(*k, 6, b, rh::KP_EMIT_L), std::memory_order_release);
      }
    }
  } catch (const std::exception& e) {
    k->dead = true;
    k->ok = false;
    k->why = e.what();
  }
  return *k;
}

rh::CompilePolicy compile_policy(int mode, uint64_t n) {
  if (mode == RH_KERNEL_SPECIALIZED) return rh::CP_BLOCKING;
  static const bool sync = [] { const char* e = std::getenv("RUHVRO_HIP_SYNC_COMPILE"); return e && *e && *e != '0'; }();
  if (n >= spec_min_records()) return sync ? rh::CP_BLOCKING : rh::CP_BACKGROUND;
  return rh::CP_CACHED_ONLY;
}

int launch_module(hipFunction_t f, const rh::KParams& P, uint32_t grid, uint32_t block, uint32_t lds, hipStream_t stream,
                  hipEvent_t start, hipEvent_t stop) {
  rh::KParams copy = P;
  void* args[] = {&copy};
  if (!start && !stop) return (int)hipModuleLaunchKernel(f, grid, 1, 1, block, 1, 1, lds, stream, args, nullptr);
  return (int)hipExtModuleLaunchKernel(f, grid * block, 1, 1, block, 1, 1, lds, stream, args, nullptr, start, stop, 0);
}

std::string format_error(const rh::ErrInfo& e) {
  char buf[128];
  switch (e.code) {
    case rh::E_EOB: return "unexpected end of buffer";
    case rh::E_VARINT: return "zigzag varint too long";
    case rh::E_EOB_F32: return "unexpected end of buffer (f32)";
    case rh::E_EOB_F64: return "unexpected end of buffer (f64)";
    case rh::E_BOOL: std::snprintf(buf, sizeof buf, "invalid boolean byte: %lld", (long long)e.detail); return buf;
    case rh::E_NEGLEN: return "negative string length";
    case rh::E_EOB_STR: return "unexpected end of buffer (string)";
    case rh::E_ENUM: std::snprintf(buf, sizeof buf, "enum index %llu out of range", (unsigned long long)e.detail); return buf;
    case rh::E_BRANCH: std::snprintf(buf, sizeof buf, "invalid union branch index: %lld", (long long)e.detail); return buf;
    case rh::E_UNION: std::snprintf(buf, sizeof buf, "union branch index out of range: %lld", (long long)e.detail); return buf;
    case rh::E_LIST_RANGE:
      std::snprintf(buf, sizeof buf, "array/map block count %lld of zero-width items exceeds the supported range", (long long)e.detail);
      return buf;
    case rh::E_INTERNAL: return "internal error: the fast and the careful walk disagree on a record";
    case rh::E_EOB_FIXED: return "unexpected end of buffer (fixed)";
    case rh::E_DECIMAL: std::snprintf(buf, sizeof buf, "decimal value of %lld bytes does not fit Decimal128", (long long)e.detail); return buf;
    case rh::E_UUID: return "invalid uuid string";
    case rh::E_DURATION: std::snprintf(buf, sizeof buf, "duration with %lld months has no value in Duration(ms)", (long long)e.detail); return buf;
    default: return "decode error";
  }
}


}
```

pyruhvro_amd/csrc/engine_pools.cpp:

```cpp
#include "engine_internal.h"

#include <sched.h>
#include <unistd.h>

#include <cctype>
#include <map>

#include <cmath>
#include <fstream>

namespace rhe {

Pool& dev_pool() { static Pool* p = new Pool(false); return *p; }
Pool& pin_pool() { static Pool* p = new Pool(true); return *p; }
CtrlPool& ctrl_pool() { static CtrlPool* p = new CtrlPool(); return *p; }

std::atomic<uint64_t> g_counters[RH_CTR_COUNT];
std::atomic<uint64_t> g_lean_counters[LC_COUNT];

char* dup_msg(const std::string& s) {
  char* p = (char*)std::malloc(s.size() + 1);
  if (p) std::memcpy(p, s.c_str(), s.size() + 1);
  return p;
}


namespace {
struct Refill {
  std::mutex mu;
  std::condition_variable cv;
  std::vector<std::pair<uint64_t, int>> queue;
  uint64_t queued_bytes = 0;
  bool started = false;
};
Refill& refill() { static Refill* r = new Refill; return *r; }
}

void Pool::prefetch(uint64_t size, int device, uint64_t budget_left) {
  if (!host_) return;
  size = align_up(std::max<uint64_t>(size, 1), 1 << 16);
  {
    const int key = pin_key(device);
    std::lock_guard<std::mutex> g(mu_);
    for (const Block& b : free_)
      if (b.device == key && b.size >= size && b.size <= size * 2 + (1 << 20)) return;
  }
  Refill& r = refill();
  std::lock_guard<std::mutex> g(r.mu);
  if (r.queued_bytes + size > budget_left || r.queue.size() >= 64) return;
  r.queue.emplace_back(size, device);
  r.queued_bytes += size;
  if (!r.started) {
    r.started = true;
    std::thread([this] {
      Refill& q = refill();
      for (;;) {
        std::pair<uint64_t, int> job;
        {
          std::unique_lock<std::mutex> l(q.mu);
          q.cv.wait(l, [&] { return !q.queue.empty(); });
          job = q.queue.front();
          q.queue.erase(q.queue.begin());
        }
        Block b;
        b.size = job.first;
        b.device = job.second;
        (void)hipSetDevice(job.second);
        b.device = pin_key(job.second);
        if (hipHostMalloc(&b.p, b.size, kPinnedFlags) == hipSuccess) put(b);
        else (void)hipGetLastError();
        std::lock_guard<std::mutex> l(q.mu);
        q.queued_bytes -= job.first;
      }
    }).detach();
  }
  r.cv.notify_one();
}

const std::vector<std::vector<int>>& numa_node_cpus() {
  static const std::vector<std::vector<int>> cached = [] {
  std::vector<std::vector<int>> nodes;
  for (int nd = 0; nd < 64; nd++) {
    FILE* f = std::fopen(("/sys/devices/system/node/node" + std::to_string(nd) + "/cpulist").c_str(), "r");
    if (!f) break;
    char buf[4096];
    std::vector<int> cpus;
    if (std::fgets(buf, sizeof buf, f)) {
      for (char* p = buf; *p;) {
        char* e = nullptr;
        const long a = std::strtol(p, &e, 10);
        if (e == p) break;
        long z = a;
        p = e;
        if (*p == '-') { z = std::strtol(p + 1, &e, 10); p = e; }
        for (long c = a; c <= z; c++) cpus.push_back((int)c);
        if (*p == ',') p++;
      }
    }
    std::fclose(f);
    nodes.push_back(cpus);
  }
// ... 78 lines not shown
```

pyruhvro_amd/csrc/rtc_compile.cpp:

```cpp
#include "rtc_compile.h"

#include <dlfcn.h>

#include <cstdio>
#include <cstdlib>
#include <cstring>
#include <mutex>
#include <stdexcept>

#include "embedded_headers.inc"

namespace rh {

namespace {
uint64_t fnv1a(const std::string& s, uint64_t h = 1469598103934665603ull) {
  for (unsigned char ch : s) { h ^= ch; h *= 1099511628211ull; }
  return h;
}
}

std::string kernel_cache_key(const std::string& source, bool encode) {
  uint64_t h = fnv1a(source);
  h = fnv1a(kHdr_program_h, h);
  h = fnv1a(kHdr_walk_h, h);
  h = fnv1a(kHdr_kernel_common_h, h);
  if (encode) {
    h = fnv1a(kHdr_encode_h, h);
    h = fnv1a(kHdr_encode_walk_h, h);
    h = fnv1a(kHdr_encode_spec_h, h);
  } else {
    h = fnv1a(kHdr_spec_body_h, h);
    if (source.find("#include \"walk_drop.h\"") != std::string::npos) h = fnv1a(kHdr_walk_drop_h, h);
    if (source.find("#include \"spec_flat.h\"") != std::string::npos) h = fnv1a(kHdr_spec_flat_h, h);
    if (source.find("#include \"walk_resolve.h\"") != std::string::npos) h = fnv1a(kHdr_walk_resolve_h, h);
  }
  char buf[32];
  std::snprintf(buf, sizeof buf, "%016llx", (unsigned long long)h);
  return buf;
}

namespace {

struct Rtc {
  void* h = nullptr;
  int (*create)(void**, const char*, const char*, int, const char* const*, const char* const*) = nullptr;
  int (*compile)(void*, int, const char* const*) = nullptr;
  int (*log_size)(void*, size_t*) = nullptr;
  int (*log)(void*, char*) = nullptr;
  int (*code_size)(void*, size_t*) = nullptr;
  int (*code)(void*, char*) = nullptr;
  int (*destroy)(void**) = nullptr;
  std::string why;
};

Rtc& rtc() {
  static Rtc r;
  static std::once_flag once;
  std::call_once(once, [] {
    const char* names[] = {"libhiprtc.so.7", "libhiprtc.so", "/opt/rocm/lib/libhiprtc.so"};
    for (const char* n : names) {
      r.h = dlopen(n, RTLD_NOW | RTLD_LOCAL);
      if (r.h) break;
    }
    if (!r.h) { r.why = std::string("hiprtc not found: ") + dlerror(); return; }
    auto sym = [&](const char* n) { return dlsym(r.h, n); };
    r.create = (decltype(r.create))sym("hiprtcCreateProgram");
    r.compile = (decltype(r.compile))sym("hiprtcCompileProgram");
    r.log_size = (decltype(r.log_size))sym("hiprtcGetProgramLogSize");
    r.log = (decltype(r.log))sym("hiprtcGetProgramLog");
    r.code_size = (decltype(r.code_size))sym("hiprtcGetCodeSize");
    r.code = (decltype(r.code))sym("hiprtcGetCode");
    r.destroy = (decltype(r.destroy))sym("hiprtcDestroyProgram");
    if (!r.create || !r.compile || !r.log_size || !r.log || !r.code_size || !r.code || !r.destroy) {
      r.why = "hiprtc symbols missing";
      r.h = nullptr;
    }
  });
  return r;
}

}

std::string module_dir() {
  Dl_info info;
  if (dladdr((void*)&kernel_cache_dir, &info) && info.dli_fname) {
    std::string p = info.dli_fname;
    size_t s = p.rfind('/');
    if (s != std::string::npos) return p.substr(0, s);
  }
  return ".";
}

std::string kernel_cache_dir() {
  if (const char* e = std::getenv("RUHVRO_HIP_KERNEL_CACHE")) return e;
  return module_dir() + "/_kcache";
}

std::vector<char> compile_kernel(const std::string& source, std::string& log) {
  Rtc& r = rtc();
  if (!r.h) throw std::runtime_error("cannot specialise the decode kernel: " + r.why);
  const char* hdr_src[] = {kHdr_program_h, kHdr_walk_h, kHdr_kernel_common_h, kHdr_spec_body_h,
                           kHdr_encode_h, kHdr_encode_walk_h, kHdr_encode_spec_h, kHdr_walk_drop_h, kHdr_spec_flat_h, kHdr_walk_resolve_h};
  const char* hdr_name[] = {"program.h", "walk.h", "kernel_common.h", "spec_body.h", "encode.h", "encode_walk.h", "encode_spec.h", "walk_drop.h", "spec_flat.h", "walk_resolve.h"};
  void* prog = nullptr;
  if (r.create(&prog, source.c_str(), "ruhvro_spec.hip", 10, hdr_src, hdr_name) != 0)
    throw std::runtime_error("hiprtcCreateProgram failed");
  const char* opts[] = {"--offload-arch=gfx950", "-O3", "-std=c++17", "-w"};
  const int rc = r.compile(prog, 4, opts);
  size_t ls = 0;
  r.log_size(prog, &ls);
  if (ls > 1) {
    log.resize(ls);
    r.log(prog, &log[0]);
  }
  if (rc != 0) {
    r.destroy(&prog);
    throw std::runtime_error("hiprtc failed to compile the specialised kernel:\n" + log);
  }
  size_t sz = 0;
  r.code_size(prog, &sz);
  std::vector<char> code(sz);
  r.code(prog, code.data());
  r.destroy(&prog);
  return code;
}

}
```

pyruhvro_amd/csrc/specialize.cpp:

```cpp
#include "specialize.h"

#include <dlfcn.h>
#include <sys/stat.h>
#include <unistd.h>

#include <algorithm>
#include <cstdio>
#include <cstdlib>
#include <cstring>
#include <fstream>
#include <map>
#include <mutex>
#include <sstream>

#include "rtc_compile.h"
#include "walk_resolve.h"

namespace rh {

namespace {

const char* op_name(int code) {
  switch (code) {
    case OP_FIXED: return "OP_FIXED";
    case OP_STRING: return "OP_STRING";
    case OP_ENUM: return "OP_ENUM";
    case OP_REC_BEGIN: return "OP_REC_BEGIN";
    case OP_REC_END: return "OP_REC_END";
    case OP_UNION_BEGIN: return "OP_UNION_BEGIN";
    case OP_VARIANT: return "OP_VARIANT";
    case OP_BIN: return "OP_BIN";
    case OP_UNION_END: return "OP_UNION_END";
    case OP_LIST_BEGIN: return "OP_LIST_BEGIN";
    case OP_LIST_NEXT: return "OP_LIST_NEXT";
    case OP_LIST_TAIL: return "OP_LIST_TAIL";
    case OP_LIST_END: return "OP_LIST_END";
    default: return "OP_END";
  }
}

}

int spec_tile_records(const CompiledSchema& cs) { return cs.wide ? kWideTile : spec_tile_records(); }

int spec_tile_records() {
  static const int v = [] {
    const char* e = std::getenv("RUHVRO_HIP_TILE");
    const int t = e ? std::atoi(e) : 256;
    return (t == 64 || t == 128 || t == 256 || t == 512 || t == 1024) ? t : 256;
  }();
  return v;
}

static thread_local bool t_lean = false;

static void emit_variant_defines(std::ostringstream& o) {
  const char* e = std::getenv("RUHVRO_HIP_VARIANT");
  std::vector<std::string> names;
  std::string name;
  for (const char* p = e ? e : "";; p++) {
    if (*p == ',' || *p == 0) {
      bool ok = !name.empty();
      for (char ch : name) ok = ok && ((ch >= 'A' && ch <= 'Z') || (ch >= '0' && ch <= '9') || ch == '_');
      if (ok) names.push_back(name);
      name.clear();
      if (*p == 0) break;
    } else {
      name.push_back(*p);
    }
  }
  if (t_lean)
    for (const char* n : {"LEN16", "INT28"})
      if (std::find(names.begin(), names.end(), n) == names.end()) names.push_back(n);
  for (const std::string& n : names) o << "#define RH_V_" << n << " 1\n";
}

static bool variant_on(const char* name) {
  if (t_lean && (!std::strcmp(name, "LEN16") || !std::strcmp(name, "INT28"))) return true;
  const char* e = std::getenv("RUHVRO_HIP_VARIANT");
  if (!e) return false;
  const std::string all = std::string(",") + e + ",";
  return all.find(std::string(",") + name + ",") != std::string::npos;
}

static std::map<size_t, int> dense_lists(const CompiledSchema& cs) {
  std::map<size_t, int> out;
  static const bool off = [] { const char* e = std::getenv("RUHVRO_HIP_NO_DENSE"); return e && *e && *e != '0'; }();
  if (off) return out;
  for (size_t i = 0; i < cs.prog.size(); i++) {
    const Op& p = cs.prog[i];
    if (p.code == OP_END) break;
    if (p.code != OP_LIST_BEGIN || p.dom != 0 || p.c != 0 || (p.flags & F_DROP)) continue;
    bool leaf = true;
    size_t j = i + 1;
    for (; j < cs.prog.size() && cs.prog[j].code != OP_LIST_END; j++)
      if (cs.prog[j].code == OP_LIST_BEGIN) { leaf = false; break; }
    if (leaf && j < cs.prog.size() && cs.prog[i + 1].code == OP_LIST_NEXT) {
      const int id = (int)out.size();
      out[i] = id;
    }
  }
  return out;
}

int dense_list_count(const CompiledSchema& cs) { return (int)dense_lists(cs).size(); }

std::string generate_kernel_source(const CompiledSchema& cs, unsigned parts) {
  std::ostringstream o;
  o << "// generated by ruhvro_hip specialize.cpp -- do not edit\n";
  emit_variant_defines(o);
  if (const char* e = std::getenv("RUHVRO_HIP_PROFILE"))
    if (*e && *e != '0') o << "#define RH_PROFILE 1\n";
  if (cs.wide) o << "#define RH_WIDE_SCHEMA 1\n";
  if (cs.max_nest > kShallowNest || cs.max_union_depth > kShallowUnionDepth) o << "#define RH_DEEP 1\n";
  o << "#include \"spec_body.h\"\n";
  if (cs.projected) o << "#include \"walk_drop.h\"\n";
  if (cs.resolved) o << "#include \"walk_resolve.h\"\n";
  const bool flat = cs.K == 0 && !cs.size_always;
  if (flat) o << "#include \"spec_flat.h\"\n";
  o << "namespace rh {\n";
  o << "struct Spec {\n";
  o << "  static constexpr int TILE = " << spec_tile_records(cs) << ";   // records (= threads) per workgroup\n";
  o << "  static constexpr int K = " << cs.K << ", KL = " << cs.KL << ", NDOM = " << cs.ndom << ", NBUF = " << cs.bufs.size()
    << ", NNODES = " << cs.nodes.size() << ", DEPTH = " << cs.list_depth << ";\n";
  o << "  static constexpr int databuf(int k) {\n    switch (k) {\n";
  for (size_t b = 0; b < cs.bufs.size(); b++)
    if (cs.bufs[b].kind == BK_DATA) o << "      case " << cs.bufs[b].counter << ": return " << b << ";\n";
  o << "      default: return 0;\n    }\n  }\n";
  {
    std::vector<int> bm;
    for (size_t b = 0; b < cs.bufs.size(); b++)
      if (cs.bufs[b].kind == BK_BITMAP && cs.bufs[b].dom != 0) bm.push_back((int)b);
    o << "  static constexpr int NBM = " << bm.size() << ";\n";
    o << "  static constexpr int bmslot(int buf) {\n    switch (buf) {\n";
    for (size_t i = 0; i < bm.size(); i++) o << "      case " << bm[i] << ": return " << i << ";\n";
    o << "      default: return 0;\n    }\n  }\n";
    o << "  static constexpr int bmbuf(int slot) {\n    switch (slot) {\n";
    for (size_t i = 0; i < bm.size(); i++) o << "      case " << i << ": return " << bm[i] << ";\n";
    o << "      default: return 0;\n    }\n  }\n";
    o << "  static constexpr int bmdom(int slot) {\n    switch (slot) {\n";
    for (size_t i = 0; i < bm.size(); i++) o << "      case " << i << ": return " << cs.bufs[bm[i]].dom << ";\n";
    o << "      default: return 1;\n    }\n  }\n";
  }
  {
    std::vector<int> b0;
    for (size_t b = 0; b < cs.bufs.size(); b++)
      if (cs.bufs[b].kind == BK_BITMAP && cs.bufs[b].dom == 0) b0.push_back((int)b);
    o << "  static constexpr int NB0 = " << b0.size() << ";\n";
    o << "  static constexpr int bm0slot(int buf) {\n    switch (buf) {\n";
    for (size_t i = 0; i < b0.size(); i++) o << "      case " << b0[i] << ": return " << i << ";\n";
    o << "      default: return 0;\n    }\n  }\n";
    o << "  static constexpr int bm0buf(int slot) {\n    switch (slot) {\n";
    for (size_t i = 0; i < b0.size(); i++) o << "      case " << i << ": return " << b0[i] << ";\n";
    o << "      default: return 0;\n    }\n  }\n";
  }
  const std::map<size_t, int> dense = dense_lists(cs);
  o << "  static constexpr int NDENSE = " << dense.size() << ";\n";
  o << "  static constexpr bool dense_body(int list, int k) {\n    switch (list) {\n";
  for (const auto& kv : dense) {
    o << "      case " << kv.second << ": return false";
    for (size_t j = kv.first + 1; cs.prog[j].code != OP_LIST_END; j++)
      if (cs.prog[j].code == OP_STRING || cs.prog[j].code == OP_ENUM) o << " || k == " << cs.prog[j].a;
    o << ";\n";
  }
  o << "      default: return false;\n    }\n  }\n";
  o << "  static constexpr int dense_str(int list) {\n    switch (list) {\n";
  for (const auto& kv : dense) {
    const size_t b = kv.first + 2;
    if (b + 1 < cs.prog.size() && cs.prog[b].code == OP_STRING && !(cs.prog[b].flags & F_NULLABLE) && cs.prog[b + 1].code == OP_LIST_TAIL)
      o << "      case " << kv.second << ": return " << cs.prog[b].a << ";\n";
  }
  o << "      default: return -1;\n    }\n  }\n";
  o << "  static __device__ __forceinline__ bool enum_sym(int b, uint32_t v, uint32_t& len, uint64_t& bits) {\n";
  if (!std::getenv("RUHVRO_HIP_NO_ENUM_IMM")) {
    std::map<int, int> seen;
    for (const Op& p : cs.prog)
      if (p.code == OP_ENUM && !(p.flags & F_DROP)) seen[p.b] = p.c;
    for (const auto& kv : seen) {
      const int b = kv.first, ns = kv.second;
      bool small = ns >= 1 && ns <= 16;
      for (int i = 0; small && i < ns; i++) small = cs.sym_off[(size_t)b + i + 1] - cs.sym_off[(size_t)b + i] <= 8;
      if (!small) continue;
      std::ostringstream ls, bs;
      uint32_t longest = 0;
      bool same_len = true;
      for (int i = 0; i < ns; i++) {
        const uint32_t l = cs.sym_off[(size_t)b + i + 1] - cs.sym_off[(size_t)b + i];
        longest = std::max(longest, l);
        same_len = same_len && l == cs.sym_off[(size_t)b + 1] - cs.sym_off[(size_t)b];
      }
      const char* suf = longest <= 4 ? "u" : "ull";
      for (int i = 0; i < ns; i++) {
        const uint32_t a0 = cs.sym_off[(size_t)b + i], a1 = cs.sym_off[(size_t)b + i + 1];
        uint64_t bits = 0;
        for (uint32_t j = a0; j < a1; j++) bits |= (uint64_t)cs.sym_data[j] << (8 * (j - a0));
        if (i + 1 < ns) { ls << "v == " << i << "u ? " << (a1 - a0) << "u : "; bs << "v == " << i << "u ? 0x" << std::hex << bits << std::dec << suf << " : "; }
        else { ls << (a1 - a0) << "u"; bs << "0x" << std::hex << bits << std::dec << suf; }
      }
      if (same_len) { ls.str(""); ls << longest << "u"; }
      o << "    if (b == " << b << ") { len = " << ls.str() << "; bits = (uint64_t)(" << bs.str() << "); return true; }\n";
    }
  }
// ... 167 lines not shown
      if (cs.wide) o << pad() << "h_topup(c, src, L);\n";
      for (int j = 0; j < rn.period; j++) {
        const Op& q0 = cs.prog[i + (size_t)j], & q1 = cs.prog[i + (size_t)rn.period + (size_t)j];
        auto fld = [&](int v0, int v1) { std::ostringstream f; f << v0; if (v1 != v0) f << " + r * " << (v1 - v0); return f.str(); };
        o << pad() << "{ const Op op = {" << op_name(q0.code) << ", " << q0.flags << ", " << q0.dom << ", " << fld(q0.a, q1.a) << ", " << fld(q0.b, q1.b)
          << ", " << q0.c << ", " << fld(q0.buf0, q1.buf0) << ", " << fld(q0.buf1, q1.buf1) << ", " << fld(q0.buf2, q1.buf2) << ", " << fld(q0.node, q1.node) << "}; ";
        const char* targs = (q0.flags & F_DROP) ? "<false, CAREFUL>(dc, src, L, op); }\n" : "<EMIT, CAREFUL>(c, src, L, op); }\n";
        switch (q0.code) {
          case OP_FIXED: o << ((q0.flags & F_PROMOTE_MASK) ? "h_fixed_p" : "h_fixed") << targs; break;
          case OP_BIN: o << "h_bin" << targs; break;
          default: o << "h_string" << targs; break;
        }
      }
      indent--;
      o << pad() << "}\n";
      i += (size_t)rn.period * rn.reps - 1;
      continue;
    }
    std::ostringstream lit;
    lit << "{" << op_name(p.code) << ", " << p.flags << ", " << p.dom << ", " << p.a << ", " << p.b << ", " << p.c << ", "
        << p.buf0 << ", " << p.buf1 << ", " << p.buf2 << ", " << p.node << "}";
    const std::string decl = "constexpr Op op = " + lit.str() + "; ";
    if (p.code == OP_LIST_NEXT && dense.count(i - 1)) {
      size_t end = i + 1;
      while (cs.prog[end].code != OP_LIST_TAIL) end++;
      o << pad() << "if constexpr (!EMIT && !CAREFUL && Ctx::kDense && Src::kSlide) {\n";
      indent++;
      o << pad() << "auto body = [&](auto em, const auto& cc, Lane& LL) {\n";
      indent++;
      for (size_t j = i + 1; j < end; j++) o << pad() << leaf_call(cs.prog[j], "false", "false", "cc", "LL");
      indent--;
      o << pad() << "};\n";
      o << pad() << "giant_list_size<Spec, " << dense.at(i - 1) << ", " << (p.a - 1) << ", " << p.c << ">(c, src, L, body);\n";
      indent--;
      o << pad() << "}\n";
      o << pad() << "if constexpr (EMIT && !CAREFUL && Ctx::kDense) {\n";
      indent++;
      o << pad() << "auto body = [&](auto em, const auto& cc, Lane& LL) {\n";
      indent++;
      o << pad() << "constexpr bool E = decltype(em)::value != 0;\n";
      for (size_t j = i + 1; j < end; j++) o << pad() << leaf_call(cs.prog[j], "E", "false", "cc", "LL");
      indent--;
      o << pad() << "};\n";
      o << pad() << "dense_list<Spec, " << dense.at(i - 1) << ", " << (p.a - 1) << ", " << p.c << ">(c, src, L, body);\n";
      indent--;
      o << pad() << "} else\n";
    }
    const bool dr = (p.flags & F_DROP) != 0;
    const std::string E = dr ? "false" : "EMIT", cx = dr ? "dc" : "c";
    const std::string tp = "<" + E + ", CAREFUL" + (la[i] ? ", " + std::to_string(la[i]) : std::string()) + ">";
    if (p.flags & F_CONST) {
      o << pad() << "{ " << decl << "run_const<EMIT, CAREFUL>(c, src, L, op); }\n";
    } else
    switch (p.code) {
      case OP_FIXED: o << pad() << "{ " << decl << ((p.flags & F_PROMOTE_MASK) ? "h_fixed_p" : "h_fixed") << tp << "(" << cx << ", src, L, op); }\n"; break;
      case OP_STRING:
      case OP_ENUM: o << pad() << "{ " << decl << "h_string" << tp << "(" << cx << ", src, L, op); }\n"; break;
      case OP_REC_BEGIN: o << pad() << "{ " << decl << "h_rec_begin" << tp << "(" << cx << ", src, L, op); }\n"; break;
      case OP_REC_END: o << pad() << "h_rec_end(L);\n"; break;
      case OP_UNION_BEGIN: o << pad() << "{ " << decl << "h_union_begin" << tp << "(" << cx << ", src, L, op); }\n"; break;
      case OP_VARIANT: o << pad() << "{ " << decl << "h_variant(L, op); }\n"; break;
      case OP_BIN: o << pad() << "{ " << decl << "h_bin<" << E << ", CAREFUL>(" << cx << ", src, L, op); }\n"; break;
      case OP_UNION_END: o << pad() << "h_union_end(L);\n"; break;
      case OP_LIST_BEGIN: o << pad() << "{ " << decl << "h_list_begin" << tp << "(" << cx << ", src, L, op); }\n"; break;
      case OP_LIST_NEXT:
        o << pad() << "for (;;) {\n";
        indent++;
        o << pad() << "{ " << decl << "if (!h_list_next<CAREFUL, (EMIT && !CAREFUL)>(" << cx << ", src, L, op)) break; }\n";
        break;
      case OP_LIST_TAIL:
        o << pad() << "{ " << decl << "h_list_tail(" << cx << ", L, op); }\n";
        indent--;
        o << pad() << "}\n";
        break;
      case OP_LIST_END: o << pad() << "{ " << decl << "h_list_end<" << E << ">(" << cx << ", L, op); }\n"; break;
      default: break;
    }
    if (p.code == OP_LIST_NEXT) list_depth++;
    if (p.code == OP_LIST_TAIL) list_depth--;
    if (cs.wide && list_depth == 0 && (p.code == OP_FIXED || p.code == OP_STRING || p.code == OP_ENUM || p.code == OP_BIN || p.code == OP_LIST_END) &&
        (++leaves % topup_every) == 0)
      o << pad() << "h_topup(c, src, L);\n";
  }
  o << "  }\n};\n";
  if (parts & (1u << KP_SIZE))
  o << "extern \"C\" __global__ void __launch_bounds__(" << spec_tile_records(cs) << ") rh_spec_size(KParams P) { spec_size<Spec>(P); }\n";
  if (parts & (1u << KP_EMIT))
    o << "extern \"C\" __global__ void __launch_bounds__(" << spec_tile_records(cs) << ") __attribute__((amdgpu_waves_per_eu(4, 8))) rh_spec_emit(KParams P) { " << (flat ? "spec_emit_flat" : "spec_emit") << "<Spec>(P); }\n";
  if (cs.K <= 64 && (parts & (1u << KP_FUSED)))
    o << "extern \"C\" __global__ void __launch_bounds__(" << spec_tile_records(cs) << ") __attribute__((amdgpu_waves_per_eu(4, 8))) rh_spec_fused(KParams P) { spec_fused<Spec>(P); }\n";
  if (parts & (1u << KP_SIZE_R))
    o << "extern \"C\" __global__ void __launch_bounds__(" << spec_tile_records(cs) << ") rh_spec_size_r(KParams P) { spec_size<Spec, true>(P); }\n";
  if (parts & (1u << KP_EMIT_R))
    o << "extern \"C\" __global__ void __launch_bounds__(" << spec_tile_records(cs) << ") __attribute__((amdgpu_waves_per_eu(" << (cs.wide ? "2, 4" : "4, 8")
      << "))) rh_spec_emit_r(KParams P) { " << (flat ? "spec_emit_flat" : "spec_emit") << "<Spec, true>(P); }\n";
  o << "}  // namespace rh\n";
  return o.str();
}

namespace {
bool enc_loads(int code) {
  return code == OP_FIXED || code == OP_STRING || code == OP_ENUM || code == OP_REC_BEGIN || code == OP_UNION_BEGIN ||
         code == OP_LIST_BEGIN || code == OP_BIN;
}
constexpr int kEncFetchBatch = 4;
constexpr int kEncLoadGroup = 32;
}

std::string generate_encode_source(const CompiledSchema& cs, unsigned parts) {
  std::ostringstream o;
  o << "// generated by ruhvro_hip specialize.cpp (encode) -- do not edit\n";
  emit_variant_defines(o);
  bool profile = false;
  if (const char* e = std::getenv("RUHVRO_HIP_PROFILE"))
    if (*e && *e != '0') profile = true;
  if (profile) o << "#define RH_PROFILE 1\n";
  int mark = 2;
  o << "#include \"encode_spec.h\"\n";
  o << "namespace rh {\n";
  o << "struct ESpec {\n";
  o << "  static constexpr int NDOM = " << cs.ndom << ", DEPTH = " << cs.list_depth << ";\n";
  const size_t nops = cs.prog.size();
  std::vector<int> group_of(nops, -1);
  std::vector<std::vector<size_t>> groups;
  {
    std::map<int, int> open;
    for (size_t i = 0; i < nops; i++) {
      const Op& p = cs.prog[i];
      if (p.code == OP_END) break;
      if (!enc_loads(p.code)) continue;
      auto it = open.find(p.dom);
      if (it == open.end() || groups[(size_t)it->second].size() >= (size_t)kEncLoadGroup) {
        groups.emplace_back();
        open[p.dom] = (int)groups.size() - 1;
        it = open.find(p.dom);
      }
      groups[(size_t)it->second].push_back(i);
      group_of[i] = it->second;
    }
  }
  auto small_enum = [&](const Op& p) {
    bool small = p.c > 0;
    for (int sidx = 0; sidx < p.c; sidx++)
      if (cs.sym_off[(size_t)p.b + sidx + 1] - cs.sym_off[(size_t)p.b + sidx] > 16) small = false;
    return small;
  };
  std::vector<char> fetched(nops, 0);
  std::map<size_t, std::vector<size_t>> batch_at;
  for (size_t g = 0; g < groups.size(); g++) {
    std::vector<size_t> cur;
    for (size_t j : groups[g]) {
      const Op& p = cs.prog[j];
      if (p.code != OP_STRING && !(p.code == OP_ENUM && small_enum(p))) continue;
      fetched[j] = 1;
      cur.push_back(j);
      if (cur.size() == (size_t)kEncFetchBatch) { batch_at[cur.front()] = cur; cur.clear(); }
    }
    if (!cur.empty()) batch_at[cur.front()] = cur;
  }
  o << "  template <int MODE, class Ctx>\n";
  o << "  static __device__ __forceinline__ void walk(Ctx& c, ELane& L) {\n";
  for (size_t i = 0; i < nops; i++) {
    const Op& p = cs.prog[i];
    if (p.code == OP_END) break;
    o << "    constexpr Op op" << i << " = {" << op_name(p.code) << ", " << p.flags << ", " << p.dom << ", " << p.a << ", "
      << p.b << ", " << p.c << ", " << p.buf0 << ", " << p.buf1 << ", " << p.buf2 << ", " << p.node << "};\n";
  }
// ... 84 lines not shown
        break;
      case OP_ENUM: {
        if (!fetched[i]) {
          o << pad() << "e_enum_put<MODE>(c, L, op" << i << ", v" << i << ", " << i
            << ", EnumTableFinder{c.sym_off, c.sym_data, op" << i << ".b, op" << i << ".c});\n";
          break;
        }
        o << pad() << "e_enum_put_pf<MODE>(c, L, op" << i << ", v" << i << ", " << i << ", d" << i
          << ", [](const v4w a, uint32_t n) -> int32_t {\n";
        indent++;
        for (int sidx = 0; sidx < p.c; sidx++) {
          const uint32_t a0 = cs.sym_off[(size_t)p.b + sidx], a1 = cs.sym_off[(size_t)p.b + sidx + 1];
          const uint32_t len = a1 - a0;
          o << pad() << "if (n == " << len << "u";
          static const char* comp[] = {"a.x", "a.y", "a.z", "a.w"};
          for (uint32_t d = 0; d * 4 < len; d++) {
            uint32_t want = 0, mask = 0;
            for (uint32_t j = 0; j < 4 && d * 4 + j < len; j++) {
              want |= (uint32_t)cs.sym_data[a0 + d * 4 + j] << (8 * j);
              mask |= 0xFFu << (8 * j);
            }
            char buf[96];
            if (mask == 0xFFFFFFFFu) std::snprintf(buf, sizeof buf, " && %s == 0x%08xu", comp[d], want);
            else std::snprintf(buf, sizeof buf, " && (%s & 0x%08xu) == 0x%08xu", comp[d], mask, want);
            o << buf;
          }
          o << ") return " << sidx << ";\n";
        }
        o << pad() << "return -1;\n";
        indent--;
        o << pad() << "});\n";
        break;
      }
      case OP_REC_BEGIN: o << pad() << "e_rec_begin<MODE>(c, L, op" << i << ", v" << i << ");\n"; break;
      case OP_REC_END: o << pad() << "e_rec_end(L);\n"; break;
      case OP_UNION_BEGIN: o << pad() << "e_union_begin<MODE>(c, L, op" << i << ", v" << i << ", " << i << ");\n"; break;
      case OP_VARIANT: o << pad() << "e_variant(L, op" << i << ");\n"; break;
      case OP_UNION_END: o << pad() << "e_union_end(L);\n"; break;
      case OP_LIST_BEGIN:
        if (profile && indent == 2 && mark < 19) o << pad() << "L.clk.mark(" << mark++ << ");\n";
        o << pad() << "e_list_begin<MODE>(c, L, op" << i << ", v" << i << ");\n";
        break;
      case OP_LIST_NEXT: {
        auto pit = pipe_at_next.find(i);
        if (pit != pipe_at_next.end() && !hoisted[i - 1])
          for (size_t j : groups[(size_t)pit->second]) o << pad() << load_type(j) << " nv" << j << " = " << load_expr(j, "") << ";\n";
        o << pad() << "for (;;) {\n";
        indent++;
        o << pad() << "if (!e_list_next(c, L, op" << i << ")) break;\n";
        break;
      }
      case OP_LIST_TAIL:
        o << pad() << "e_list_tail(c, L, op" << i << ");\n";
        indent--;
        o << pad() << "}\n";
        break;
      case OP_LIST_END:
        o << pad() << "e_list_end<MODE>(c, L);\n";
        if (profile && indent == 2 && mark < 19) o << pad() << "L.clk.mark(" << mark++ << ");\n";
        break;
      default: break;
    }
  }
  if (profile) o << "    L.clk.mark(19);\n";
  o << "  }\n};\n";
  if (parts & (1u << KP_ESIZE))
    o << "extern \"C\" __global__ void __launch_bounds__(256) rh_espec_size(EParams P) {\n"
    << "  extern __shared__ __attribute__((aligned(16))) uint8_t smem[];\n  e_size_body<ESpecW<ESpec>>(P, smem);\n}\n";
  if (parts & (1u << KP_EEMIT))
    o << "extern \"C\" __global__ void __launch_bounds__(256) rh_espec_emit(EParams P) {\n"
    << "  extern __shared__ __attribute__((aligned(16))) uint8_t smem[];\n  e_emit_body<ESpecW<ESpec>>(P, smem);\n}\n";
  o << "}  // namespace rh\n";
  return o.str();
}

bool schema_has_lean(const CompiledSchema& cs) { return (cs.K > 0 || cs.size_always) && !cs.wide; }

std::string generate_lean_source(const CompiledSchema& cs, unsigned parts) {
  if (!schema_has_lean(cs)) return "";
  struct Scope { Scope() { t_lean = true; } ~Scope() { t_lean = false; } } lean;
  return generate_kernel_source(cs, parts);
}

std::string generate_part_source(const CompiledSchema& cs, int part) {
  if (part < 0 || part >= KP_COUNT) return "";
  if (part == KP_SIZE_L || part == KP_EMIT_L) return generate_lean_source(cs, 1u << (part == KP_SIZE_L ? KP_SIZE : KP_EMIT));
  if (part == KP_FUSED && cs.K > 64) return "";
  if (kernel_part_is_encode(part)) return (cs.encode_unsupported.empty() && !cs.projected) ? generate_encode_source(cs, 1u << part) : std::string();
  return generate_kernel_source(cs, 1u << part);
}

}
```

pyruhvro_amd/csrc/specialize.h:

```cpp
#pragma once
#include <string>
#include <vector>

#include "schema.h"

namespace rh {

int spec_tile_records();
int spec_tile_records(const CompiledSchema& cs);
enum KernelPart { KP_SIZE = 0, KP_EMIT = 1, KP_FUSED = 2, KP_ESIZE = 3, KP_EEMIT = 4, KP_SIZE_R = 5, KP_EMIT_R = 6, KP_SIZE_L = 7, KP_EMIT_L = 8, KP_COUNT = 9 };
constexpr unsigned kDecodeParts = 7u | 96u, kEncodeParts = 24u, kLeanParts = (1u << KP_SIZE_L) | (1u << KP_EMIT_L);
inline bool kernel_part_is_encode(int part) { return part == KP_ESIZE || part == KP_EEMIT; }
inline const char* kernel_part_entry(int part) {
  static const char* const names[KP_COUNT] = {"rh_spec_size", "rh_spec_emit", "rh_spec_fused", "rh_espec_size", "rh_espec_emit", "rh_spec_size_r", "rh_spec_emit_r", "rh_spec_size", "rh_spec_emit"};
  return names[part];
}
std::string generate_kernel_source(const CompiledSchema& cs, unsigned parts = kDecodeParts);
std::string generate_encode_source(const CompiledSchema& cs, unsigned parts = kEncodeParts);
bool schema_has_lean(const CompiledSchema& cs);
std::string generate_lean_source(const CompiledSchema& cs, unsigned parts = kDecodeParts);
std::string generate_part_source(const CompiledSchema& cs, int part);

inline uint32_t spec_lds_fixed_words_host(int K, int nnodes, int nw, int nbm, int ndense, int nb0) {
  return (((uint32_t)(K > 0 ? K : 1) + 3) & ~3u) * (uint32_t)(nw + 1) + 128u + (uint32_t)((nnodes + 3) & ~3) + (uint32_t)((nnodes * nw + 3) & ~3) + 4 + (uint32_t)(nbm * 64) +
         (ndense > 0 ? (uint32_t)(nw * 128) : 0u) + (((uint32_t)(nb0 * nw * 2) + 3) & ~3u);
}
inline int dom0_bitmap_count(const CompiledSchema& cs) {
  int n = 0;
  for (const BufDesc& d : cs.bufs) n += (d.kind == BK_BITMAP && d.dom == 0) ? 1 : 0;
  return n;
}
int dense_list_count(const CompiledSchema& cs);
inline int child_bitmap_count(const CompiledSchema& cs) {
  int n = 0;
  for (const BufDesc& d : cs.bufs) n += (d.kind == BK_BITMAP && d.dom != 0) ? 1 : 0;
  return n;
}

}
```

pyruhvro_amd/prebuild.py:

```python
from __future__ import annotations

import os
import sys
from concurrent.futures import ProcessPoolExecutor
from typing import Iterable, List, Tuple


def _one(item) -> Tuple[bool, str]:
    from pyruhvro_amd import cabi
    try:
        if isinstance(item, tuple) and len(item) == 3 and item[0] == "resolve":
            return cabi.prebuild(item[1], reader_schema=item[2]), ""
        if isinstance(item, tuple):
            return cabi.prebuild(item[0], columns=item[1]), ""
        return cabi.prebuild(item), ""
    except Exception as e:
        return False, str(e)


def _cache_dir() -> str:
    return os.environ.get("RUHVRO_HIP_KERNEL_CACHE") or os.path.join(os.path.dirname(os.path.abspath(__file__)), "_kcache")


def _marker(schemas: List[str]) -> str:
    import hashlib
    variant = os.environ.get("RUHVRO_HIP_VARIANT", "")
    h = hashlib.sha1(("\0".join(sorted(s if isinstance(s, str) else repr(s) for s in schemas)) + "\1" + variant).encode()).hexdigest()[:16]
    return os.path.join(_cache_dir(), f"warm_{h}.ok")


def cache_looks_warm(schemas: Iterable[str]) -> bool:
    return os.path.exists(_marker(list(dict.fromkeys(schemas))))


def prebuild_many(schemas: Iterable[str], jobs: int = 0, verbose: bool = False) -> List[str]:
    uniq = list(dict.fromkeys(schemas))
    jobs = jobs or max(1, min(len(uniq), (os.cpu_count() or 2) // 2, 16))
    os.environ.setdefault("RUHVRO_HIP_COMPILE_JOBS", "2")
    errors: List[str] = []
    if not uniq:
        return errors
    if jobs <= 1:
        results = [_one(s) for s in uniq]
    else:
        with ProcessPoolExecutor(max_workers=jobs) as ex:
            results = list(ex.map(_one, uniq))
    hits = sum(1 for hit, err in results if hit and not err)
    for (hit, err), s in zip(results, uniq):
        if err:
            errors.append(err)
    if not errors:
        try:
            os.makedirs(_cache_dir(), exist_ok=True)
            open(_marker(uniq), "w").close()
        except OSError:
            pass
    if verbose:
        print(f"kernel cache: {len(uniq)} schemas, {hits} already cached, {len(uniq) - hits - len(errors)} compiled, "
              f"{len(errors)} failed")
    return errors


def mark_warm(schemas: Iterable[str]) -> None:
    try:
        os.makedirs(_cache_dir(), exist_ok=True)
        open(_marker(list(dict.fromkeys(schemas))), "w").close()
    except OSError:
        pass


def benchmark_schemas() -> List[str]:
    root = os.path.dirname(os.path.dirname(os.path.abspath(__file__)))
    if root not in sys.path:
        sys.path.insert(0, root)
    from avrogen.schemas import SCHEMAS
    return list(SCHEMAS.values())


if __name__ == "__main__":
    os.environ.setdefault("RUHVRO_HIP_PREBUILD_LEAN", "1")
    errs = prebuild_many(benchmark_schemas(), verbose=True)
    for e in errs:
        print(e[:2000])
    sys.exit(1 if errs else 0)
```

Baseline: 9.775 billion.

## Add notes-based single-pass fused decode kernel with automatic selection

Adds a new specialized fused decode kernel variant (spec_notes.h) that records per-record notes during a walk pass and replays them in the emit pass, so the source does not need to be fully re-parsed. For large batches (at least 4M records) on schemas whose lean state is clean, it is auto-selected in place of the two-pass path, with fallback and learning from dirty tiles. Prebuild now compiles the notes kernel too. It adds kernel-compile cost and extra register pressure, and it falls back when tiles need careful handling.

```diff
diff --git a/include/ruhvro_hip.h b/include/ruhvro_hip.h
--- a/include/ruhvro_hip.h
+++ b/include/ruhvro_hip.h
@@ -116,6 +116,11 @@
   RH_LEAN_COUNT = 11
 };
 uint32_t rh_lean_counters(uint64_t* out, uint32_t n);
+
+char* rh_schema_notes_kernel_source(const rh_schema* s);
+char* rh_schema_notes_kernel_key(const rh_schema* s);
+int rh_schema_has_notes(const rh_schema* s);
+uint32_t rh_notes_counters(uint64_t* out, uint32_t n);
 
 int rh_encode(const rh_schema* s, const struct ArrowArray* batch, const struct ArrowSchema* batch_schema,
               uint64_t num_chunks, const rh_opts* opts, struct ArrowArray* out_chunks, uint32_t* out_k,
diff --git a/pyruhvro_amd/_build.py b/pyruhvro_amd/_build.py
--- a/pyruhvro_amd/_build.py
+++ b/pyruhvro_amd/_build.py
@@ -13,7 +13,7 @@
 LIB_SOURCES = ["kernels.hip", "encode.hip", "validate.hip", "container.hip", "engine_tolerant.cpp", "engine_container.cpp", "container_scan.cpp", "engine.cpp", "engine_pools.cpp", "engine_kernels.cpp", "engine_device_call.cpp", "engine_host.cpp",
                "engine_export.cpp", "engine_encode.cpp", "schema.cpp", "specialize.cpp", "rtc_compile.cpp", "kernel_jobs.cpp"]
 HELPER = os.path.join(HERE, "rh_kcompile")
-EMBED = ["program.h", "walk.h", "kernel_common.h", "spec_body.h", "encode.h", "encode_walk.h", "encode_spec.h", "walk_drop.h", "spec_flat.h", "walk_resolve.h"]
+EMBED = ["program.h", "walk.h", "kernel_common.h", "spec_body.h", "encode.h", "encode_walk.h", "encode_spec.h", "walk_drop.h", "spec_flat.h", "walk_resolve.h", "spec_notes.h"]
 LIB_DEPS = LIB_SOURCES + EMBED + ["engine_internal.h", "specialize.h", "rtc_compile.h", "kernel_jobs.h", "kcompile_main.cpp", "schema.h", "validate.h", "container.h", "container_scan.h", "json.hpp", "../../include/ruhvro_hip.h", "../../include/arrow_c_abi.h"]
 
 
diff --git a/pyruhvro_amd/cabi.py b/pyruhvro_amd/cabi.py
--- a/pyruhvro_amd/cabi.py
+++ b/pyruhvro_amd/cabi.py
@@ -345,6 +345,30 @@
     return {name: int(buf[i]) for i, name in enumerate(LEAN_COUNTERS)}
 
 
+NOTES_COUNTERS = ("notes_calls", "failovers", "fallbacks")
+
+
+def notes_kernel_source(schema_json: str, columns=None, reader_schema=None):
+    return _lean_string("rh_schema_notes_kernel_source", schema_json, columns, reader_schema)
+
+
+def notes_kernel_key(schema_json: str, columns=None, reader_schema=None):
+    return _lean_string("rh_schema_notes_kernel_key", schema_json, columns, reader_schema)
+
+
+def has_notes(schema_json: str, columns=None, reader_schema=None) -> bool:
+    f = _lean_sym("rh_schema_has_notes", C.c_int, [C.c_void_p])
+    return bool(f(Schema.get(schema_json, columns, reader_schema).handle)) if f else False
+
+
+def notes_counters() -> dict:
+    f = _lean_sym("rh_notes_counters", C.c_uint32, [C.POINTER(C.c_uint64), C.c_uint32])
+    buf = (C.c_uint64 * len(NOTES_COUNTERS))()
+    if f is not None:
+        assert f(buf, len(NOTES_COUNTERS)) == len(NOTES_COUNTERS)
+    return {name: int(buf[i]) for i, name in enumerate(NOTES_COUNTERS)}
+
+
 def encode_kernel_source(schema_json: str) -> str:
     L = lib()
     p = L.rh_schema_encode_kernel_source(Schema.get(schema_json).handle)
diff --git a/pyruhvro_amd/csrc/engine.cpp b/pyruhvro_amd/csrc/engine.cpp
--- a/pyruhvro_amd/csrc/engine.cpp
+++ b/pyruhvro_amd/csrc/engine.cpp
@@ -304,6 +304,33 @@
   return (it == s->spec.end() || !it->second) ? 0 : it->second->lean_state;
 }
 
+char* rh_schema_notes_kernel_source(const rh_schema* s) {
+  if (!s) return nullptr;
+  try {
+    const std::string src = rh::generate_notes_source(*s->cs);
+    return src.empty() ? nullptr : dup_msg(src);
+  } catch (...) {
+    return nullptr;
+  }
+}
+
+char* rh_schema_notes_kernel_key(const rh_schema* s) {
+  if (!s) return nullptr;
+  try {
+    const std::string src = rh::generate_notes_source(*s->cs);
+    return src.empty() ? nullptr : dup_msg(rh::kernel_cache_key(src, false));
+  } catch (...) {
+    return nullptr;
+  }
+}
+
+int rh_schema_has_notes(const rh_schema* s) { return (s && rh::schema_has_notes(*s->cs)) ? 1 : 0; }
+
+uint32_t rh_notes_counters(uint64_t* out, uint32_t n) {
+  for (uint32_t i = 0; i < n && i < (uint32_t)NC_COUNT; i++) out[i] = g_notes_counters[i].load(std::memory_order_relaxed);
+  return NC_COUNT;
+}
+
 char* rh_schema_encode_kernel_source(const rh_schema* s) {
   if (!s || !s->cs->encode_unsupported.empty() || s->cs->projected) return nullptr;
   try {
@@ -319,9 +346,10 @@
     const bool fused = env_long("RUHVRO_HIP_PREBUILD_FUSED", 1, 0, 1) != 0;
     const bool ranged = env_long("RUHVRO_HIP_PREBUILD_RANGED", 1, 0, 1) != 0;
     const bool lean = env_long("RUHVRO_HIP_PREBUILD_LEAN", 0, 0, 1) != 0;
+    const bool notes = env_long("RUHVRO_HIP_PREBUILD_NOTES", 0, 0, 1) != 0 && rh::schema_has_notes(*s->cs);
     const unsigned parts = (rh::kDecodeParts & ~(fused ? 0u : (1u << rh::KP_FUSED)) & ~(ranged ? 0u : ((1u << rh::KP_SIZE_R) | (1u << rh::KP_EMIT_R)))) |
                            ((s->cs->encode_unsupported.empty() && !s->cs->wide && !s->cs->projected) ? rh::kEncodeParts : 0u) |
-                           (lean ? rh::kLeanParts : 0u);
+                           (lean ? rh::kLeanParts : 0u) | (notes ? (1u << rh::KP_NOTES) : 0u);
     rh::KernelImage im[rh::KP_COUNT];
     const unsigned started = rh::kernel_images(s->images, *s->cs, parts, rh::CP_BLOCKING, im);
     for (int p = 0; p < rh::KP_COUNT; p++) {
diff --git a/pyruhvro_amd/csrc/engine_device_call.cpp b/pyruhvro_amd/csrc/engine_device_call.cpp
--- a/pyruhvro_amd/csrc/engine_device_call.cpp
+++ b/pyruhvro_amd/csrc/engine_device_call.cpp
@@ -46,6 +46,8 @@
   bool child_bitmaps = false, fused = false, timed_size = false;
   bool range_of_host_call = false;
   bool single = false;
+  bool notes = false;
+  bool notes_auto = false;
   std::vector<uint64_t> caps;
   uint64_t arena_cap = 0, o_tick = 0;
   Lease lookback, hcaps;
@@ -264,7 +266,7 @@
   }
 
   void lean_learn(bool dirty) {
-    if (!lean) return;
+    if (!lean && !notes_auto) return;
     std::lock_guard<std::mutex> g(s->mu);
     SpecKernel& sl = sel();
     if (dirty) {
@@ -272,7 +274,7 @@
         sl.lean_backoff = std::min<uint32_t>(1024, std::max<uint32_t>(8, sl.lean_backoff * 2));
         sl.lean_wait = sl.lean_backoff;
         sl.lean_state = SpecKernel::LS_WIDE;
-        lean_count(LC_FALLBACKS);
+        if (lean) lean_count(LC_FALLBACKS);
       }
     } else if (sl.lean_state == SpecKernel::LS_LEAN) {
       sl.lean_backoff = 0;
@@ -281,12 +283,34 @@
 
   bool try_single(bool two_sync, long ratio_hook) {
     const bool on = (opts.flags & RH_SINGLE_PASS) != 0 || env_long("RUHVRO_HIP_SINGLE_PASS", kSinglePassDefault, 0, 1) != 0;
-    if (!on || range_of_host_call || (opts.flags & (RH_INTERNAL_TWO_PASS | RH_TWO_PASS)) || !sk || K <= 0 || K > 64 || n == 0 || two_sync ||
+    const long notes_mode = env_long("RUHVRO_HIP_NOTES", -1, 0, 1);
+    bool want_notes = false;
+    if (notes_mode != 0 && sk && !sk->notes_dead && rh::schema_has_notes(cs)) {
+      if (notes_mode == 1) {
+        want_notes = true;
+      } else if (!on) {
+        const long min_n = env_long("RUHVRO_HIP_NOTES_MIN_RECORDS", kNotesMinRecords, 0, 1l << 40);
+        if (min_n > 0 && n >= (uint64_t)min_n) {
+          std::lock_guard<std::mutex> g(s->mu);
+          want_notes = sel().lean_state == SpecKernel::LS_LEAN;
+        }
+      }
+    }
+    if ((!on && !want_notes) || range_of_host_call || (opts.flags & (RH_INTERNAL_TWO_PASS | RH_TWO_PASS)) || !sk || K <= 0 || K > 64 || n == 0 || two_sync ||
         ratio_hook >= 0)
       return false;
     if (n_entries > (1u << 16)) return false;
     if (8ull * K * k > 4ull * K * nblocks) return false;
-    hipFunction_t fused_fn = sk->fused_fn.load(std::memory_order_acquire);
+    hipFunction_t fused_fn = nullptr;
+    if (want_notes) {
+      fused_fn = sk->notes_fn.load(std::memory_order_acquire);
+      if (!fused_fn) fused_fn = spec_kernel(s, device, notes_mode == 1 ? rh::CP_BLOCKING : rh::CP_BACKGROUND, false, false, false, false, true).notes_fn.load(std::memory_order_acquire);
+      if (!fused_fn) want_notes = false;
+    }
+    if (!fused_fn) {
+      if (!on) return false;
+      fused_fn = sk->fused_fn.load(std::memory_order_acquire);
+    }
     if (!fused_fn) {
       if (sk->fused_dead) return false;
       fused_fn = spec_kernel(s, device, compile_policy(opts.flags & 3, n), false, true).fused_fn.load(std::memory_order_acquire);
@@ -320,6 +344,7 @@
         }
       arena_cap = std::max<uint64_t>(off, kAlign);
     }
+    if (want_notes) { notes = true; notes_auto = notes_mode != 1; notes_count(NC_CALLS); }
     count(RH_CTR_SINGLE_PASS_CALLS);
     count(RH_CTR_FUSED_CALLS);
     single = true; fused = true;
@@ -638,6 +663,13 @@
       if (K > 0) std::memcpy(totals.data(), hctrl.ptr() + o_tot, 8ull * K * k);
       if (single) {
         ctrl->b.clean = published;
+        if (notes && published) {
+          const uint32_t* stw = (const uint32_t*)(hctrl.ptr() + 32);
+          count(RH_CTR_CAREFUL_TILES, stw[0]); count(RH_CTR_REWALKED_WAVES, stw[2]);
+          if (stw[0] != 0 || stw[2] != 0) notes_count(NC_FALLBACKS);
+          lean_learn(stw[0] != 0 || stw[2] != 0);
+        }
+        if (notes && lflag) notes_count(NC_FAILOVERS);
         if (lflag) {
           if ((lflag & rh::LF_CAPACITY) && env_long("RUHVRO_HIP_SINGLE_SLACK_PERMILLE", 1040, 1, 4000) >= 1000) {
             std::lock_guard<std::mutex> g(s->mu);
diff --git a/pyruhvro_amd/csrc/engine_internal.h b/pyruhvro_amd/csrc/engine_internal.h
--- a/pyruhvro_amd/csrc/engine_internal.h
+++ b/pyruhvro_amd/csrc/engine_internal.h
@@ -298,7 +298,7 @@
 };
 
 struct SpecKernel {
-  hipModule_t mod[7] = {nullptr, nullptr, nullptr, nullptr, nullptr, nullptr, nullptr};
+  hipModule_t mod[8] = {nullptr, nullptr, nullptr, nullptr, nullptr, nullptr, nullptr, nullptr};
   hipFunction_t size_fn = nullptr, emit_fn = nullptr;
   std::atomic<hipFunction_t> size_r_fn{nullptr}, emit_r_fn{nullptr};
   std::atomic<bool> ranged_dead{false};
@@ -311,6 +311,8 @@
   bool lean_probing = false;
   std::atomic<hipFunction_t> fused_fn{nullptr};
   std::atomic<bool> fused_dead{false};
+  std::atomic<hipFunction_t> notes_fn{nullptr};
+  std::atomic<bool> notes_dead{false};
   std::atomic<bool> ok{false};
   std::atomic<bool> dead{false};
   std::string why;
@@ -339,7 +341,10 @@
 const DeviceProgram& device_program(rh_schema* s, int device);
 uint64_t spec_min_records();
 const SpecKernel& spec_kernel(rh_schema* s, int device, rh::CompilePolicy policy, bool encode = false, bool want_fused = false, bool want_ranged = false,
-                              bool want_lean = false);
+                              bool want_lean = false, bool want_notes = false);
+enum NotesCounter { NC_CALLS = 0, NC_FAILOVERS, NC_FALLBACKS, NC_COUNT };
+extern std::atomic<uint64_t> g_notes_counters[NC_COUNT];
+inline void notes_count(int which, uint64_t by = 1) { g_notes_counters[which].fetch_add(by, std::memory_order_relaxed); }
 enum LeanCounter { LC_LEAN_CALLS = 0, LC_PROBES, LC_PROBES_CLEAN, LC_PROBES_DIRTY, LC_FALLBACKS, LC_RERUNS, LC_NEED_RANGED, LC_NEED_WIDE_INDEX,
                    LC_TWO_PASS_REPEATS, LC_CAPACITY_TAILS, LC_ASYNC_SETTLED, LC_COUNT };
 extern std::atomic<uint64_t> g_lean_counters[LC_COUNT];
@@ -508,6 +513,7 @@
 void settle(rh_device_result* r);
 
 constexpr long kSinglePassDefault = 0;
+constexpr long kNotesMinRecords = 4000000;
 constexpr int kPublicFlags = 3 | RH_ASYNC | RH_TWO_PASS | RH_SINGLE_PASS;
 constexpr int RH_INTERNAL_HOST_ARENA = 0x200;
 constexpr int RH_INTERNAL_TWO_PASS = 0x100;
diff --git a/pyruhvro_amd/csrc/engine_kernels.cpp b/pyruhvro_amd/csrc/engine_kernels.cpp
--- a/pyruhvro_amd/csrc/engine_kernels.cpp
+++ b/pyruhvro_amd/csrc/engine_kernels.cpp
@@ -45,7 +45,7 @@
   return fn;
 }
 
-const SpecKernel& spec_kernel(rh_schema* s, int device, rh::CompilePolicy policy, bool encode, bool want_fused, bool want_ranged, bool want_lean) {
+const SpecKernel& spec_kernel(rh_schema* s, int device, rh::CompilePolicy policy, bool encode, bool want_fused, bool want_ranged, bool want_lean, bool want_notes) {
   std::map<int, std::unique_ptr<SpecKernel>>& table = encode ? s->espec : s->spec;
   SpecKernel* k = nullptr;
   {
@@ -56,12 +56,13 @@
     if (k->dead) return *k;
     if (k->ok && (!want_fused || k->fused_dead || k->fused_fn.load(std::memory_order_acquire)) &&
         (!want_ranged || k->ranged_dead || k->emit_r_fn.load(std::memory_order_acquire)) &&
-        (!want_lean || k->lean_dead || k->emit_l_fn.load(std::memory_order_acquire))) return *k;
+        (!want_lean || k->lean_dead || k->emit_l_fn.load(std::memory_order_acquire)) &&
+        (!want_notes || k->notes_dead || k->notes_fn.load(std::memory_order_acquire))) return *k;
   }
   const int p_size = encode ? rh::KP_ESIZE : rh::KP_SIZE, p_emit = encode ? rh::KP_EEMIT : rh::KP_EMIT;
   const unsigned parts = (1u << p_size) | (1u << p_emit) | ((want_fused && !encode) ? (1u << rh::KP_FUSED) : 0u) |
                          ((want_ranged && !encode) ? ((1u << rh::KP_SIZE_R) | (1u << rh::KP_EMIT_R)) : 0u) |
-                         ((want_lean && !encode) ? rh::kLeanParts : 0u);
+                         ((want_lean && !encode) ? rh::kLeanParts : 0u) | ((want_notes && !encode) ? (1u << rh::KP_NOTES) : 0u);
   rh::KernelImage im[rh::KP_COUNT];
   const unsigned started = rh::kernel_images(s->images, *s->cs, parts, policy, im);
   if (started && policy == rh::CP_BACKGROUND) g_counters[RH_CTR_BACKGROUND_COMPILES].fetch_add(started, std::memory_order_relaxed);
@@ -104,6 +105,11 @@
         k->size_l_fn.store(load_part(*k, 5, a, rh::KP_SIZE_L), std::memory_order_release);
         k->emit_l_fn.store(load_part(*k, 6, b, rh::KP_EMIT_L), std::memory_order_release);
       }
+    }
+    if (k->ok && want_notes && !encode && !k->notes_dead && !k->notes_fn.load(std::memory_order_relaxed)) {
+      const rh::KernelImage& f = im[rh::KP_NOTES];
+      if (f.state == rh::IMG_FAILED || f.state == rh::IMG_NONE) k->notes_dead = true;
+      else if (f.state == rh::IMG_READY) k->notes_fn.store(load_part(*k, 7, f, rh::KP_NOTES), std::memory_order_release);
     }
   } catch (const std::exception& e) {
     k->dead = true;
diff --git a/pyruhvro_amd/csrc/engine_pools.cpp b/pyruhvro_amd/csrc/engine_pools.cpp
--- a/pyruhvro_amd/csrc/engine_pools.cpp
+++ b/pyruhvro_amd/csrc/engine_pools.cpp
@@ -17,6 +17,7 @@
 
 std::atomic<uint64_t> g_counters[RH_CTR_COUNT];
 std::atomic<uint64_t> g_lean_counters[LC_COUNT];
+std::atomic<uint64_t> g_notes_counters[NC_COUNT];
 
 char* dup_msg(const std::string& s) {
   char* p = (char*)std::malloc(s.size() + 1);
diff --git a/pyruhvro_amd/csrc/rtc_compile.cpp b/pyruhvro_amd/csrc/rtc_compile.cpp
--- a/pyruhvro_amd/csrc/rtc_compile.cpp
+++ b/pyruhvro_amd/csrc/rtc_compile.cpp
@@ -33,6 +33,7 @@
     if (source.find("#include \"walk_drop.h\"") != std::string::npos) h = fnv1a(kHdr_walk_drop_h, h);
     if (source.find("#include \"spec_flat.h\"") != std::string::npos) h = fnv1a(kHdr_spec_flat_h, h);
     if (source.find("#include \"walk_resolve.h\"") != std::string::npos) h = fnv1a(kHdr_walk_resolve_h, h);
+    if (source.find("#include \"spec_notes.h\"") != std::string::npos) h = fnv1a(kHdr_spec_notes_h, h);
   }
   char buf[32];
   std::snprintf(buf, sizeof buf, "%016llx", (unsigned long long)h);
@@ -100,10 +101,10 @@
   Rtc& r = rtc();
   if (!r.h) throw std::runtime_error("cannot specialise the decode kernel: " + r.why);
   const char* hdr_src[] = {kHdr_program_h, kHdr_walk_h, kHdr_kernel_common_h, kHdr_spec_body_h,
-                           kHdr_encode_h, kHdr_encode_walk_h, kHdr_encode_spec_h, kHdr_walk_drop_h, kHdr_spec_flat_h, kHdr_walk_resolve_h};
-  const char* hdr_name[] = {"program.h", "walk.h", "kernel_common.h", "spec_body.h", "encode.h", "encode_walk.h", "encode_spec.h", "walk_drop.h", "spec_flat.h", "walk_resolve.h"};
+                           kHdr_encode_h, kHdr_encode_walk_h, kHdr_encode_spec_h, kHdr_walk_drop_h, kHdr_spec_flat_h, kHdr_walk_resolve_h, kHdr_spec_notes_h};
+  const char* hdr_name[] = {"program.h", "walk.h", "kernel_common.h", "spec_body.h", "encode.h", "encode_walk.h", "encode_spec.h", "walk_drop.h", "spec_flat.h", "walk_resolve.h", "spec_notes.h"};
   void* prog = nullptr;
-  if (r.create(&prog, source.c_str(), "ruhvro_spec.hip", 10, hdr_src, hdr_name) != 0)
+  if (r.create(&prog, source.c_str(), "ruhvro_spec.hip", 11, hdr_src, hdr_name) != 0)
     throw std::runtime_error("hiprtcCreateProgram failed");
   const char* opts[] = {"--offload-arch=gfx950", "-O3", "-std=c++17", "-w"};
   const int rc = r.compile(prog, 4, opts);
diff --git a/pyruhvro_amd/csrc/spec_notes.h b/pyruhvro_amd/csrc/spec_notes.h
--- /dev/null
+++ b/pyruhvro_amd/csrc/spec_notes.h
@@ -0,0 +1,425 @@
+#pragma once
+#include "spec_body.h"
+
+#if !defined(RH_V_LEN16) || !defined(RH_V_INT28)
+#error "spec_notes.h: the note packing is that of the narrow single-read forms (RH_V_LEN16, RH_V_INT28)"
+#endif
+
+namespace rh {
+
+template <int NV, int NM>
+struct Notes {
+  uint32_t v[NV > 0 ? NV : 1];
+  uint32_t m[NM > 0 ? NM : 1];
+  __device__ __forceinline__ void clear() {
+    static_for<0, (NV > 0 ? NV : 1)>([&](auto i) { v[decltype(i)::value] = 0; });
+    static_for<0, (NM > 0 ? NM : 1)>([&](auto i) { m[decltype(i)::value] = 0; });
+  }
+  template <int VB> __device__ __forceinline__ void put(bool b) { if constexpr (VB >= 0) m[VB / 32] |= (b ? 1u : 0u) << (VB % 32); }
+  template <int VB> __device__ __forceinline__ bool get(bool dflt) const {
+    if constexpr (VB >= 0) return ((m[VB / 32] >> (VB % 32)) & 1u) != 0;
+    else return dflt;
+  }
+};
+
+template <int SLOT, int VB, int LA, class Src, class Ctx, class NT>
+__device__ __forceinline__ void n_fixed(const Ctx& c, const Src& src, Lane& L, const Op& op, NT& nt) {
+  const bool dec = L.live && L.pres;
+  const bool is_int = op.a == FK_I32 || op.a == FK_I64;
+  int64_t v = 0;
+  const bool isval = read_head<false, false, LA>(src, L, dec, (op.flags & F_NULLABLE) != 0, (op.flags & F_NULL_FIRST) != 0, is_int, op.a == FK_I64, v);
+  uint64_t bits;
+  bool valid;
+  if (is_int) {
+    valid = isval && L.live;
+    bits = op.a == FK_I32 ? (uint64_t)(uint32_t)(int32_t)v : (uint64_t)v;
+  } else {
+    uint64_t x;
+    if constexpr ((LA & 1) != 0) x = L.la;
+    else if constexpr ((LA & 2) != 0 && (LA >> 2) == 8) x = src.ld8(L.cur);
+    else if constexpr ((LA & 2) != 0) x = (uint64_t)src.ld4(L.cur);
+    else x = op.a == FK_F64 ? src.ld8(L.cur) : op.a == FK_F32 ? src.ld5(L.cur) : (uint64_t)src.ld1(L.cur);
+    const uint32_t need = op.a == FK_F32 ? 4u : op.a == FK_F64 ? 8u : 1u;
+    const bool want = isval && L.live;
+    bits = op.a == FK_F32 ? (uint64_t)(uint32_t)x : op.a == FK_F64 ? x : (x & 0xFFu);
+    L.redo = L.redo || (want && op.a == FK_BOOL && bits > 1);
+    valid = want;
+    L.cur += valid ? need : 0u;
+    if constexpr ((LA & 2) != 0) L.la = x >> (8u * (valid ? need : 0u));
+  }
+  if (!valid) bits = 0;
+  nt.v[SLOT] = (uint32_t)bits;
+  if (op.a == FK_I64 || op.a == FK_F64) nt.v[SLOT + 1] = (uint32_t)(bits >> 32);
+  nt.template put<VB>(valid);
+}
+
+template <int SLOT, int VB, int LA, class Src, class Ctx, class NT>
+__device__ __forceinline__ void n_string(const Ctx& c, const Src& src, Lane& L, const Op& op, NT& nt) {
+  const bool dec = L.live && L.pres;
+  int64_t v = 0;
+  const bool isval = read_head<false, false, LA>(src, L, dec, (op.flags & F_NULLABLE) != 0, (op.flags & F_NULL_FIRST) != 0, true, false, v, op.code == OP_STRING ? 2 : 1);
+  const bool want = isval && L.live;
+  uint32_t len = 0;
+  if (op.code == OP_STRING) {
+    len = want ? (uint32_t)v : 0u;
+    L.redo = L.redo || (want && (L.cur >> 16) != 0u);
+    nt.v[SLOT] = (L.cur & 0xFFFFu) | (len << 16);
+    nt.template put<VB>(want);
+    L.cur += len;
+  } else {
+    const bool oor = want && (uint32_t)v >= (uint32_t)op.c;
+    reject<false>(L, oor, E_ENUM, v);
+    const bool has = want && L.live;
+    uint64_t sym_bits = 0;
+    uint32_t l0 = 0;
+    if (c.enum_sym(op.b, (uint32_t)v, l0, sym_bits)) {
+      len = has ? l0 : 0u;
+    } else if (has) {
+      const uint32_t spos = c.sym_off[op.b + (int32_t)v];
+      len = c.sym_off[op.b + (int32_t)v + 1] - spos;
+    }
+    nt.v[SLOT] = ((uint32_t)v & 0x7FFFFFFFu) | (has ? 0x80000000u : 0u);
+    nt.template put<VB>(has);
+  }
+  c.counter(op.a) += len;
+}
+
+template <int VB, int LA, class Src, class Ctx, class NT>
+__device__ __forceinline__ void n_rec_begin(const Ctx& c, const Src& src, Lane& L, const Op& op, NT& nt) {
+  L.pstk = (L.pstk << 1) | (stk_t)(L.pres ? 1u : 0u);
+  const bool dec = L.live && L.pres;
+  int64_t dummy = 0;
+  const bool isval = read_head<false, false, LA>(src, L, dec, true, (op.flags & F_NULL_FIRST) != 0, false, false, dummy);
+  const bool valid = isval && L.live;
+  nt.template put<VB>(valid);
+  L.pres = valid;
+}
+
+template <int SLOT, int LA, class Src, class Ctx, class NT>
+__device__ __forceinline__ void n_union_begin(const Ctx& c, const Src& src, Lane& L, const Op& op, NT& nt) {
+  L.pstk = (L.pstk << 1) | (stk_t)(L.pres ? 1u : 0u);
+  L.sstk = (L.sstk << 8) | (sel_t)0xFFull;
+  const bool dec = L.live && L.pres;
+  int64_t idx = 0;
+  const bool got = read_head<false, false, LA>(src, L, dec, false, false, true, false, idx, 1) && L.live;
+  const bool oor = got && (uint32_t)idx >= (uint32_t)op.a;
+  reject<false>(L, oor, E_UNION, idx);
+  uint32_t tidv = 0;
+  if (got && L.live) { tidv = (uint32_t)idx; L.sstk = (L.sstk & ~(sel_t)0xFFull) | (sel_t)(uint64_t)idx; }
+  nt.v[SLOT] = tidv;
+}
+
+template <int SLOT, int VB, int LA, class Src, class Ctx, class NT>
+__device__ __forceinline__ void n_list_begin(const Ctx& c, const Src& src, Lane& L, const Op& op, NT& nt) {
+  L.pstk = (L.pstk << 1) | (stk_t)(L.pres ? 1u : 0u);
+  L.lstk = (L.lstk << 1) | (stk_t)(L.live ? 1u : 0u);
+  const bool dec = L.live && L.pres;
+  int64_t dummy = 0;
+  const bool isval = read_head<false, false, LA>(src, L, dec, (op.flags & F_NULLABLE) != 0, (op.flags & F_NULL_FIRST) != 0, false, false, dummy);
+  const bool valid = isval && L.live;
+  nt.template put<VB>(valid);
+  nt.v[SLOT] = L.cur;
+  L.live = valid;
+  L.pres = valid;
+  c.remaining(op.c) = 0;
+}
+
+template <int SLOT, int VB, class Ctx, class NT>
+__device__ __forceinline__ void e_fixed(const Ctx& c, const Lane& L, const Op& op, const NT& nt) {
+  const bool act = L.live;
+  const bool valid = nt.template get<VB>(act);
+  const uint32_t row = c.lrow;
+  if (op.a == FK_BOOL) {
+    c.template put_word0<false>(op.buf1, __ballot(nt.v[SLOT] != 0));
+  } else {
+    void* const pf1 = c.buf(op.buf1);
+    if (act) {
+      if (op.a == FK_I32 || op.a == FK_F32) st_global<uint32_t, Ctx::kWide>(pf1, row, nt.v[SLOT]);
+      else st_global<uint64_t, Ctx::kWide>(pf1, row, ((uint64_t)nt.v[SLOT + 1] << 32) | nt.v[SLOT]);
+    }
+  }
+  put_validity<true, false>(c, op, act, valid, row);
+}
+
+template <int SLOT, int VB, class Src, class Ctx, class NT>
+__device__ __forceinline__ void e_string(const Ctx& c, const Src& src, const Lane& L, const Op& op, const NT& nt) {
+  const bool act = L.live;
+  void* const pb1 = c.buf(op.buf1);
+  void* const pb2 = c.buf(op.buf2);
+  const uint32_t note = nt.v[SLOT];
+  const uint32_t row = c.lrow;
+  const uint32_t o = c.counter(op.a), gb = c.gbase(op.a);
+  bool valid;
+  if (op.code == OP_STRING) {
+    const uint32_t len = note >> 16, spos = note & 0xFFFFu;
+    valid = nt.template get<VB>(act);
+    if (act) {
+      st_global<uint32_t, Ctx::kWide>(pb1, row + 1, gb + o + len);
+      if (len) copy_bytes<Ctx::kWide>(pb2, (typename BufOff<Ctx::kWide>::type)gb + o, src, spos, len);
+    }
+  } else {
+    valid = (note >> 31) != 0;
+    uint32_t len = 0, spos = 0;
+    if (valid) {
+      const uint32_t v = note & 0x7FFFFFFFu;
+      spos = c.sym_off[op.b + (int32_t)v];
+      len = c.sym_off[op.b + (int32_t)v + 1] - spos;
+    }
+    if (act) {
+      st_global<uint32_t, Ctx::kWide>(pb1, row + 1, gb + o + len);
+      if (len) {
+        RH_GLOBAL uint8_t* d = reinterpret_cast<RH_GLOBAL uint8_t*>(reinterpret_cast<uintptr_t>(pb2)) + gb + o;
+        copy_plain(d, c.sym_data + spos, len);
+      }
+    }
+  }
+  put_validity<true, false>(c, op, act, valid, row);
+}
+
+template <int VB, class Ctx, class NT>
+__device__ __forceinline__ void e_rec_begin(const Ctx& c, const Lane& L, const Op& op, const NT& nt) {
+  put_validity<true, false>(c, op, L.live, nt.template get<VB>(L.live), c.lrow);
+}
+
+template <int SLOT, class Ctx, class NT>
+__device__ __forceinline__ void e_union_begin(const Ctx& c, const Lane& L, const Op& op, const NT& nt) {
+  void* const pu1 = c.buf(op.buf1);
+  if (L.live) st_global<int8_t, Ctx::kWide>(pu1, c.lrow, (int8_t)nt.v[SLOT]);
+}
+
+template <int SLOT, int VB, class Ctx, class NT>
+__device__ __forceinline__ void e_list_begin(const Ctx& c, Lane& L, const Op& op, const NT& nt) {
+  const bool act = L.live;
+  const bool valid = nt.template get<VB>(false);
+  L.pstk = (L.pstk << 1) | (stk_t)(L.pres ? 1u : 0u);
+  L.lstk = (L.lstk << 1) | (stk_t)(L.live ? 1u : 0u);
+  put_validity<true, false>(c, op, act, valid, c.lrow);
+  L.cur = nt.v[SLOT];
+  L.live = valid;
+  L.pres = valid;
+  c.remaining(op.c) = 0;
+}
+
+template <class S>
+__device__ __forceinline__ void spec_fused_notes(const KParams& P) {
+  extern __shared__ __attribute__((aligned(16))) uint8_t smem[];
+  if (reinterpret_cast<const uint32_t*>(P.first_bad)[2] != 0) return;
+  const SpecSmem<S> s(P, smem);
+  const uint32_t tid = threadIdx.x, lane = tid & 63, wave = tid >> 6;
+  RH_MARK_INIT;
+  constexpr int T = TileOf<S>::T, NW = TileOf<S>::NW, KP = SCtx<S>::KP;
+  static_assert(S::K > 0 && S::K <= 64 && S::KL == S::K, "the notes part is for schemas with a size pass that are not wide");
+#ifndef RH_V_NOPRIO
+  __builtin_amdgcn_s_setprio(3);
+#endif
+  const uint32_t chunk = blockIdx.x % P.k;
+  const uint64_t rows_c = chunk == P.k - 1 ? P.rows_last : P.sz;
+  const uint32_t tiles_c = (uint32_t)((rows_c + T - 1) / T);
+  if (blockIdx.x / P.k >= tiles_c) return;
+  if (tid == 0) {
+    s.misc[3] = __hip_atomic_fetch_add(&P.tickets[chunk], 1u, __ATOMIC_RELAXED, __HIP_MEMORY_SCOPE_AGENT);
+    s.misc[0] = 0xFFFFFFFFu; s.misc[1] = 0; s.misc[2] = 0;
+  }
+  for (int i = tid; i < S::NNODES; i += T) s.nullcnt[i] = 0;
+  for (int i = tid; i < S::NNODES * NW; i += T) s.nullw[i] = 0;
+  for (int i = tid; i < S::NBM * kBmWords; i += T) s.bm[i] = 0;
+  __syncthreads();
+  RH_MARK(0);
+  const uint32_t lb = s.misc[3];
+  const uint32_t tile = chunk * P.bpc + lb;
+  Geo g;
+  g.chunk = chunk; g.lrow0 = lb * T; g.rec0 = (uint64_t)chunk * P.sz + g.lrow0;
+  { const uint64_t left = rows_c - g.lrow0; g.nrec = left < (uint64_t)T ? (uint32_t)left : (uint32_t)T; }
+  uint64_t o0 = 0, o1 = 0;
+  if (tid < g.nrec) { o0 = P.offsets[g.rec0 + tid]; o1 = P.offsets[g.rec0 + tid + 1]; }
+  const uint64_t wb = P.offsets[g.rec0], we = P.offsets[g.rec0 + g.nrec];
+  const uint64_t wb16 = wb & ~15ull;
+  const bool fits = (we - wb16) <= (uint64_t)P.win_bytes;
+  if (fits) stage_window<T>(P, s.win, wb16, we, tid);
+  __syncthreads();
+  RH_MARK(1);
+
+  Lane L;
+  SCtx<S> c;
+  Notes<S::NNOTE, S::NNMASK> nt;
+  spec_ctx_init(c, P, s, g, tid);
+  c.bufp = (const __attribute__((address_space(4))) uint64_t*)(reinterpret_cast<uintptr_t>(P.bufptr) + (size_t)chunk * S::NBUF * 8);
+  lane_init_from(L, g, o0, o1, wb16, tid);
+  if (L.live && (we - wb16) > 0xFFFFFFF0ull) L.err = E_EOB;
+  const bool noting = fits && P.all_careful == 0;
+  bool careful = !noting;
+  const uint32_t wa = (uint32_t)(uintptr_t)(RH_LDS uint8_t*)s.win;
+  if (noting) {
+    nt.clear();
+    L.cur += wa; L.end += wa;
+    S::note_walk(c, LdsAbsSrc(), L, nt);
+    L.redo = L.redo || L.cur > L.end;
+  }
+  if (!noting || __any(L.redo)) {
+    if (noting && lane == 0) atomicAdd(reinterpret_cast<uint32_t*>(P.first_bad) + 10, 1u);
+    careful = true;
+    spec_ctx_init(c, P, s, g, tid);
+    lane_init_from(L, g, o0, o1, wb16, tid);
+    if (L.live && (we - wb16) > 0xFFFFFFF0ull) L.err = E_EOB;
+    spec_run_walk<S, false, true>(P, c, s.win, L, fits, wb16);
+  }
+  RH_MARK(2);
+  if (lane == 0 && careful) atomicOr(&s.misc[2], 2u);
+  uint32_t allor = 0;
+  static_for<0, S::K>([&](auto ik) { allor |= c.cnt[decltype(ik)::value]; });
+  if (!__any(allor > 1023u)) {
+    constexpr int NDW = (S::K + 1) / 2;
+    uint32_t tot[KP] = {};
+    static_for<0, NDW>([&](auto id) {
+      constexpr int d = decltype(id)::value;
+      uint32_t v = c.cnt[2 * d];
+      if constexpr (2 * d + 1 < S::K) v |= c.cnt[2 * d + 1] << 16;
+      const uint32_t incl = wave_incl_scan(v, lane);
+      const uint32_t ex = incl - v;
+      c.cnt[2 * d] = ex & 0xFFFFu;
+      tot[2 * d] = incl & 0xFFFFu;
+      if constexpr (2 * d + 1 < S::K) { c.cnt[2 * d + 1] = ex >> 16; tot[2 * d + 1] = incl >> 16; }
+    });
+    if (lane == 63) {
+      static_for<0, KP / 4>([&](auto iq) {
+        constexpr int q = decltype(iq)::value;
+        v4w x; x.x = tot[4 * q]; x.y = tot[4 * q + 1]; x.z = tot[4 * q + 2]; x.w = tot[4 * q + 3];
+        *reinterpret_cast<v4w*>(s.wtot + wave * KP + 4 * q) = x;
+      });
+    }
+  } else {
+    static_for<0, S::K>([&](auto ik) {
+      constexpr int k = decltype(ik)::value;
+      const uint32_t v = c.cnt[k];
+      const uint32_t incl = wave_incl_scan(v, lane);
+      if (lane == 63) s.wtot[wave * KP + k] = incl;
+      c.cnt[k] = incl - v;
+    });
+  }
+  if (L.err) atomicMin(&s.misc[0], tid);
+  RH_MARK(3);
+  __syncthreads();
+  RH_MARK(4);
+  if (s.misc[0] == tid) {
+    ErrInfo ei; ei.code = L.err; ei.pad = 0; ei.detail = L.edetail;
+    P.errinfo[tile] = ei;
+    atomicMax(P.first_bad, ~(unsigned long long)(g.rec0 + tid));
+  }
+  careful = careful || (s.misc[2] & 2u) != 0 || s.misc[0] != 0xFFFFFFFFu;
+  if (tid == 0 && careful && P.all_careful == 0) atomicAdd(reinterpret_cast<uint32_t*>(P.first_bad) + 8, 1u);
+
+  if (wave == 0) {
+    constexpr uint32_t NJ = 64 / S::K;
+    const uint32_t k_of = lane % (uint32_t)S::K, j_of = lane / (uint32_t)S::K;
+    const bool in_grid = j_of < NJ;
+    uint32_t agg = 0;
+    if (lane < (uint32_t)S::K)
+      for (int w = 0; w < NW; w++) agg += s.wtot[w * KP + lane];
+    unsigned long long* const mine = P.lookback + (size_t)tile * S::K + k_of;
+    if (lane < (uint32_t)S::K)
+      __hip_atomic_store(mine, (lb == 0 ? kLbInc : kLbAgg) | agg, __ATOMIC_RELAXED, __HIP_MEMORY_SCOPE_AGENT);
+    uint32_t excl = 0;
+    bool found = lb == 0, stuck = false;
+    uint32_t* const xw = s.gbx + KP;
+    for (uint32_t back = 1;; back += NJ) {
+      if (!__any(lane < (uint32_t)S::K && !found)) break;
+      uint32_t val = 0, st = 2;
+      const uint32_t dist = back + j_of;
+      if (in_grid && dist <= lb) {
+        const unsigned long long* q = mine - (size_t)dist * S::K;
+        unsigned long long w = __hip_atomic_load(q, __ATOMIC_RELAXED, __HIP_MEMORY_SCOPE_AGENT);
+        for (uint32_t spins = 0; (w >> 62) == 0 && spins < (1u << 24); spins++) {
+          __builtin_amdgcn_s_sleep(1);
+          w = __hip_atomic_load(q, __ATOMIC_RELAXED, __HIP_MEMORY_SCOPE_AGENT);
+        }
+        if ((w >> 62) == 0) { stuck = true; w = kLbInc; }
+        val = (uint32_t)w; st = (uint32_t)(w >> 62);
+      }
+      if (in_grid) { xw[2 * lane] = val; xw[2 * lane + 1] = st; }
+      __builtin_amdgcn_fence(__ATOMIC_ACQ_REL, "wavefront");
+      if (lane < (uint32_t)S::K && !found) {
+        for (uint32_t j = 0; j < NJ && !found; j++) {
+          excl += xw[2 * (j * S::K + lane)];
+          found = xw[2 * (j * S::K + lane) + 1] == 2u;
+        }
+      }
+      __builtin_amdgcn_fence(__ATOMIC_ACQ_REL, "wavefront");
+    }
+    uint32_t over = 0;
+    if (lane < (uint32_t)S::K) {
+      if (lb != 0) __hip_atomic_store(mine, kLbInc | (unsigned long long)(uint32_t)(excl + agg), __ATOMIC_RELAXED, __HIP_MEMORY_SCOPE_AGENT);
+      const uint64_t end = (uint64_t)excl + agg;
+      over = end > P.caps[(size_t)lane * P.k + chunk] ? 1u : 0u;
+      if (lb == tiles_c - 1) P.totals[(size_t)lane * P.k + chunk] = end;
+      s.gbx[lane] = excl;
+    }
+    if (__any(over != 0 || stuck)) {
+      if (lane == 0) {
+        s.misc[1] = 1;
+        atomicOr(reinterpret_cast<uint32_t*>(P.first_bad) + 2, (uint32_t)LF_CAPACITY);
+      }
+    }
+  }
+  RH_MARK(5);
+  __syncthreads();
+  RH_MARK(6);
+  if (s.misc[1] != 0) return;
+  static_for<0, S::K>([&](auto ik) {
+    constexpr int k = decltype(ik)::value;
+    c.gb[k] = (uint32_t)__builtin_amdgcn_readfirstlane((int)s.gbx[k]);
+  });
+  if constexpr (NW > 1) {
+    uint32_t prev = 0;
+    if (lane < (uint32_t)S::K) {
+      for (int w = 0; w < NW - 1; w++) prev += (int)wave > w ? s.wtot[w * KP + lane] : 0u;
+    }
+    static_for<0, S::K>([&](auto ik) {
+      constexpr int k = decltype(ik)::value;
+      c.cnt[k] += (uint32_t)__builtin_amdgcn_readlane((int)prev, k);
+    });
+  }
+
+#ifndef RH_V_NOPRIO
+  __builtin_amdgcn_s_setprio(0);
+#endif
+  RH_MARK(7);
+  if (careful) {
+    lane_init_from(L, g, o0, o1, wb16, tid);
+    if (L.live && (we - wb16) > 0xFFFFFFF0ull) L.err = E_EOB;
+    spec_run_walk<S, true, true>(P, c, s.win, L, fits, wb16);
+  } else {
+    lane_init_from(L, g, o0, o1, wb16, tid);
+    L.cur += wa; L.end += wa;
+    S::note_emit(c, LdsAbsSrc(), L, nt);
+    if (L.redo) L.err = E_INTERNAL;
+  }
+  RH_MARK(8);
+  if (tid == 0) s.misc[0] = 0xFFFFFFFFu;
+  __syncthreads();
+  report_errors(P, s.misc, L, g, tid, tile);
+  for (int i = tid; i < S::NNODES; i += T) {
+    uint32_t v = s.nullcnt[i];
+    for (int w = 0; w < NW; w++) v += s.nullw[i * NW + w];
+    if (v) atomicAdd(&P.nullcount[((size_t)i * P.k + g.chunk) * P.null_slots + (tile & (P.null_slots - 1))], v);
+  }
+  if constexpr (S::NB0 > 0) {
+    for (uint32_t i = tid; i < (uint32_t)(S::NB0 * NW); i += T) {
+      const uint32_t slot = i / NW, w = i % NW;
+      if (w * 64u < g.nrec) st_global<uint64_t, false>(c.buf(S::bm0buf(slot)), (g.lrow0 >> 6) + w, c.bmw0[i]);
+    }
+  }
+  if constexpr (S::NBM > 0) {
+    static_for<0, S::NBM>([&](auto ib) {
+      constexpr int slot = decltype(ib)::value;
+      const uint32_t w0 = c.gb[S::bmdom(slot) - 1] >> 5;
+      for (int w = tid; w < kBmWords; w += T) {
+        const uint32_t v = s.bm[slot * kBmWords + w];
+        if (v) atomic_or_global(c.buf(S::bmbuf(slot)), (uint64_t)w0 + w, v);
+      }
+    });
+  }
+  RH_MARK(9);
+  RH_MARK_FLUSH;
+}
+
+}
diff --git a/pyruhvro_amd/csrc/specialize.cpp b/pyruhvro_amd/csrc/specialize.cpp
--- a/pyruhvro_amd/csrc/specialize.cpp
+++ b/pyruhvro_amd/csrc/specialize.cpp
@@ -53,6 +53,39 @@
 }
 
 static thread_local bool t_lean = false;
+static thread_local bool t_notes = false;
+
+namespace {
+struct NoteAt { int slot = -1, vb = -1; };
+bool notes_layout(const CompiledSchema& cs, std::vector<NoteAt>& at, int& nslots, int& nbits) {
+  at.assign(cs.prog.size(), NoteAt());
+  nslots = nbits = 0;
+  int depth = 0;
+  bool any = false;
+  for (size_t i = 0; i < cs.prog.size() && cs.prog[i].code != OP_END; i++) {
+    const Op& p = cs.prog[i];
+    if ((p.flags & (F_DROP | F_CONST | F_PROMOTE_MASK | F_WAVE_CTR)) || p.code == OP_BIN) return false;
+    if (p.code == OP_LIST_NEXT) { depth++; continue; }
+    if (p.code == OP_LIST_TAIL) { depth--; continue; }
+    if (depth > 0) {
+      if (p.code == OP_LIST_BEGIN) return false;
+      continue;
+    }
+    if (p.dom != 0) return false;
+    const bool nb = (p.flags & F_CAN_NULL) != 0;
+    switch (p.code) {
+      case OP_FIXED: at[i].slot = nslots; nslots += (p.a == FK_I64 || p.a == FK_F64) ? 2 : 1; if (nb) at[i].vb = nbits++; any = true; break;
+      case OP_STRING: at[i].slot = nslots++; if (nb) at[i].vb = nbits++; any = true; break;
+      case OP_ENUM: at[i].slot = nslots++; any = true; break;
+      case OP_REC_BEGIN: at[i].vb = nbits++; break;
+      case OP_UNION_BEGIN: at[i].slot = nslots++; any = true; break;
+      case OP_LIST_BEGIN: at[i].slot = nslots++; at[i].vb = nbits++; break;
+      default: break;
+    }
+  }
+  return any && nslots <= 40 && nbits <= 64;
+}
+}
 
 static void emit_variant_defines(std::ostringstream& o) {
   const char* e = std::getenv("RUHVRO_HIP_VARIANT");
@@ -118,6 +151,7 @@
   if (cs.resolved) o << "#include \"walk_resolve.h\"\n";
   const bool flat = cs.K == 0 && !cs.size_always;
   if (flat) o << "#include \"spec_flat.h\"\n";
+  if (t_notes) o << "#include \"spec_notes.h\"\n";
   o << "namespace rh {\n";
   o << "struct Spec {\n";
   o << "  static constexpr int TILE = " << spec_tile_records(cs) << ";   // records (= threads) per workgroup\n";
@@ -451,7 +485,112 @@
         (++leaves % topup_every) == 0)
       o << pad() << "h_topup(c, src, L);\n";
   }
-  o << "  }\n};\n";
+  o << "  }\n";
+  if (t_notes) {
+    std::vector<NoteAt> at;
+    int nslots = 0, nbits = 0;
+    notes_layout(cs, at, nslots, nbits);
+    o << "  static constexpr int NNOTE = " << nslots << ", NNMASK = " << (nbits + 31) / 32 << ";\n";
+    auto decl_of = [&](const Op& p) {
+      std::ostringstream lit;
+      lit << "constexpr Op op = {" << op_name(p.code) << ", " << p.flags << ", " << p.dom << ", " << p.a << ", " << p.b << ", " << p.c << ", "
+          << p.buf0 << ", " << p.buf1 << ", " << p.buf2 << ", " << p.node << "}; ";
+      return lit.str();
+    };
+    for (int emit = 0; emit < 2; emit++) {
+      const std::string E = emit ? "true" : "false";
+      o << "  template <class Src, class Ctx, class NT>\n";
+      o << "  static __device__ __forceinline__ void " << (emit ? "note_emit" : "note_walk") << "(const Ctx& c, const Src& src, Lane& L, "
+        << (emit ? "const NT& nt" : "NT& nt") << ") {\n";
+      int depth = 0;
+      indent = 2;
+      for (size_t i = 0; i < cs.prog.size() && cs.prog[i].code != OP_END; i++) {
+        const Op& p = cs.prog[i];
+        const std::string sl = std::to_string(at[i].slot), vb = std::to_string(at[i].vb), las = std::to_string(la[i]);
+        const std::string d = "{ " + decl_of(p);
+        if (p.code == OP_LIST_NEXT) {
+          size_t end = i + 1;
+          while (cs.prog[end].code != OP_LIST_TAIL) end++;
+          if (emit && dense.count(i - 1)) {
+            o << pad() << "{\n";
+            indent++;
+            o << pad() << "auto body = [&](auto em, const auto& cc, Lane& LL) {\n";
+            indent++;
+            o << pad() << "constexpr bool E = decltype(em)::value != 0;\n";
+            for (size_t j = i + 1; j < end; j++) o << pad() << leaf_call(cs.prog[j], "E", "false", "cc", "LL");
+            indent--;
+            o << pad() << "};\n";
+            o << pad() << "dense_list<Spec, " << dense.at(i - 1) << ", " << (p.a - 1) << ", " << p.c << ">(c, src, L, body);\n";
+            indent--;
+            o << pad() << "}\n";
+            i = end;
+            continue;
+          }
+          o << pad() << "for (;;) {\n";
+          indent++;
+          o << pad() << d << "if (!h_list_next<false, " << E << ">(c, src, L, op)) break; }\n";
+          depth++;
+          continue;
+        }
+        if (p.code == OP_LIST_TAIL) {
+          o << pad() << d << "h_list_tail(c, L, op); }\n";
+          indent--;
+          o << pad() << "}\n";
+          depth--;
+          continue;
+        }
+        if (depth > 0) {
+          const std::string tp = "<" + E + ", false" + (la[i] ? ", " + las : std::string()) + ">";
+          switch (p.code) {
+            case OP_FIXED: o << pad() << d << "h_fixed" << tp << "(c, src, L, op); }\n"; break;
+            case OP_STRING:
+            case OP_ENUM: o << pad() << d << "h_string" << tp << "(c, src, L, op); }\n"; break;
+            case OP_REC_BEGIN: o << pad() << d << "h_rec_begin" << tp << "(c, src, L, op); }\n"; break;
+            case OP_REC_END: o << pad() << "h_rec_end(L);\n"; break;
+            case OP_UNION_BEGIN: o << pad() << d << "h_union_begin" << tp << "(c, src, L, op); }\n"; break;
+            case OP_VARIANT: o << pad() << d << "h_variant(L, op); }\n"; break;
+            case OP_UNION_END: o << pad() << "h_union_end(L);\n"; break;
+            default: break;
+          }
+          continue;
+        }
+        switch (p.code) {
+          case OP_FIXED:
+            if (emit) o << pad() << d << "e_fixed<" << sl << ", " << vb << ">(c, L, op, nt); }\n";
+            else o << pad() << d << "n_fixed<" << sl << ", " << vb << ", " << las << ">(c, src, L, op, nt); }\n";
+            break;
+          case OP_STRING:
+          case OP_ENUM:
+            if (emit) o << pad() << d << "e_string<" << sl << ", " << vb << ">(c, src, L, op, nt); }\n";
+            else o << pad() << d << "n_string<" << sl << ", " << vb << ", " << las << ">(c, src, L, op, nt); }\n";
+            break;
+          case OP_REC_BEGIN:
+            if (emit) o << pad() << d << "e_rec_begin<" << vb << ">(c, L, op, nt); }\n";
+            else o << pad() << d << "n_rec_begin<" << vb << ", " << las << ">(c, src, L, op, nt); }\n";
+            break;
+          case OP_REC_END: if (!emit) o << pad() << "h_rec_end(L);\n"; break;
+          case OP_UNION_BEGIN:
+            if (emit) o << pad() << d << "e_union_begin<" << sl << ">(c, L, op, nt); }\n";
+            else o << pad() << d << "n_union_begin<" << sl << ", " << las << ">(c, src, L, op, nt); }\n";
+            break;
+          case OP_VARIANT: if (!emit) o << pad() << d << "h_variant(L, op); }\n"; break;
+          case OP_UNION_END: if (!emit) o << pad() << "h_union_end(L);\n"; break;
+          case OP_LIST_BEGIN:
+            if (emit) o << pad() << d << "e_list_begin<" << sl << ", " << vb << ">(c, L, op, nt); }\n";
+            else o << pad() << d << "n_list_begin<" << sl << ", " << vb << ", " << las << ">(c, src, L, op, nt); }\n";
+            break;
+          case OP_LIST_END: o << pad() << d << "h_list_end<" << E << ">(c, L, op); }\n"; break;
+          default: break;
+        }
+      }
+      o << "  }\n";
+    }
+    o << "};\n";
+    o << "extern \"C\" __global__ void __launch_bounds__(" << spec_tile_records(cs) << ") __attribute__((amdgpu_waves_per_eu(4, 8))) rh_spec_fused(KParams P) { spec_fused_notes<Spec>(P); }\n";
+    o << "}  // namespace rh\n";
+    return o.str();
+  }
+  o << "};\n";
   if (parts & (1u << KP_SIZE))
   o << "extern \"C\" __global__ void __launch_bounds__(" << spec_tile_records(cs) << ") rh_spec_size(KParams P) { spec_size<Spec>(P); }\n";
   if (parts & (1u << KP_EMIT))
@@ -702,8 +841,23 @@
   return generate_kernel_source(cs, parts);
 }
 
+bool schema_has_notes(const CompiledSchema& cs) {
+  if (!schema_has_lean(cs) || cs.K <= 0 || cs.K > 64 || cs.KL != cs.K || cs.projected || cs.resolved || cs.list_depth > 1) return false;
+  if (cs.max_nest > kShallowNest || cs.max_union_depth > kShallowUnionDepth) return false;
+  std::vector<NoteAt> at;
+  int nslots = 0, nbits = 0;
+  return notes_layout(cs, at, nslots, nbits);
+}
+
+std::string generate_notes_source(const CompiledSchema& cs) {
+  if (!schema_has_notes(cs)) return "";
+  struct Scope { Scope() { t_lean = true; t_notes = true; } ~Scope() { t_lean = false; t_notes = false; } } notes;
+  return generate_kernel_source(cs, 0u);
+}
+
 std::string generate_part_source(const CompiledSchema& cs, int part) {
   if (part < 0 || part >= KP_COUNT) return "";
+  if (part == KP_NOTES) return generate_notes_source(cs);
   if (part == KP_SIZE_L || part == KP_EMIT_L) return generate_lean_source(cs, 1u << (part == KP_SIZE_L ? KP_SIZE : KP_EMIT));
   if (part == KP_FUSED && cs.K > 64) return "";
   if (kernel_part_is_encode(part)) return (cs.encode_unsupported.empty() && !cs.projected) ? generate_encode_source(cs, 1u << part) : std::string();
diff --git a/pyruhvro_amd/csrc/specialize.h b/pyruhvro_amd/csrc/specialize.h
--- a/pyruhvro_amd/csrc/specialize.h
+++ b/pyruhvro_amd/csrc/specialize.h
@@ -8,17 +8,19 @@
 
 int spec_tile_records();
 int spec_tile_records(const CompiledSchema& cs);
-enum KernelPart { KP_SIZE = 0, KP_EMIT = 1, KP_FUSED = 2, KP_ESIZE = 3, KP_EEMIT = 4, KP_SIZE_R = 5, KP_EMIT_R = 6, KP_SIZE_L = 7, KP_EMIT_L = 8, KP_COUNT = 9 };
+enum KernelPart { KP_SIZE = 0, KP_EMIT = 1, KP_FUSED = 2, KP_ESIZE = 3, KP_EEMIT = 4, KP_SIZE_R = 5, KP_EMIT_R = 6, KP_SIZE_L = 7, KP_EMIT_L = 8, KP_NOTES = 9, KP_COUNT = 10 };
 constexpr unsigned kDecodeParts = 7u | 96u, kEncodeParts = 24u, kLeanParts = (1u << KP_SIZE_L) | (1u << KP_EMIT_L);
 inline bool kernel_part_is_encode(int part) { return part == KP_ESIZE || part == KP_EEMIT; }
 inline const char* kernel_part_entry(int part) {
-  static const char* const names[KP_COUNT] = {"rh_spec_size", "rh_spec_emit", "rh_spec_fused", "rh_espec_size", "rh_espec_emit", "rh_spec_size_r", "rh_spec_emit_r", "rh_spec_size", "rh_spec_emit"};
+  static const char* const names[KP_COUNT] = {"rh_spec_size", "rh_spec_emit", "rh_spec_fused", "rh_espec_size", "rh_espec_emit", "rh_spec_size_r", "rh_spec_emit_r", "rh_spec_size", "rh_spec_emit", "rh_spec_fused"};
   return names[part];
 }
 std::string generate_kernel_source(const CompiledSchema& cs, unsigned parts = kDecodeParts);
 std::string generate_encode_source(const CompiledSchema& cs, unsigned parts = kEncodeParts);
 bool schema_has_lean(const CompiledSchema& cs);
 std::string generate_lean_source(const CompiledSchema& cs, unsigned parts = kDecodeParts);
+bool schema_has_notes(const CompiledSchema& cs);
+std::string generate_notes_source(const CompiledSchema& cs);
 std::string generate_part_source(const CompiledSchema& cs, int part);
 
 inline uint32_t spec_lds_fixed_words_host(int K, int nnodes, int nw, int nbm, int ndense, int nb0) {
diff --git a/pyruhvro_amd/prebuild.py b/pyruhvro_amd/prebuild.py
--- a/pyruhvro_amd/prebuild.py
+++ b/pyruhvro_amd/prebuild.py
@@ -79,6 +79,7 @@
 
 if __name__ == "__main__":
     os.environ.setdefault("RUHVRO_HIP_PREBUILD_LEAN", "1")
+    os.environ.setdefault("RUHVRO_HIP_PREBUILD_NOTES", "1")
     errs = prebuild_many(benchmark_schemas(), verbose=True)
     for e in errs:
         print(e[:2000])
```

Result: no change. 9.764 billion (-0.1%).
